# hellosunking/Microcket

Hardware: AMD Instinct MI355X
Metric: read-pairs/sec through sam2pairs+dedup (150 bp PE, hg38 names, SAM text resident in HBM) (higher is better)
Workload: dtype u8; 1 GPU; C2: 100 M 150 bp PE Micro-C read pairs, hg38, one MI355X -- 100000000 synthetic 150 bp PE read pairs per GPU, hg38 chromosome names, 1 lane(s), unc mode, sam=no, seed 20260105, one step = one pass over the whole resident data set + duplicate marking of the reported pairs on (chr1,pos1,chr2,pos2,strands) + per-chromosome-pair counts; preset=C2, pairs_per_gpu=100000001, sam_bytes_per_gpu=94584442002, block_groups=2097152, blocks=48, parallelism=shard1: independent read-group shards, no data-path collective

## Files before the change

### microcket_amd/csrc/mkt_capi.cpp

```cpp
#include "mkt_ctx.h"

extern "C" {

int mkt_abi_version(void) { return MKT_ABI_VERSION; }

const char* mkt_strerror(int code) {
    switch (code) {
    case MKT_OK: return "ok";
    case MKT_E_ARG: return "bad argument";
    case MKT_E_NO_DEVICE: return "no usable HIP device (this library has no CPU path)";
    case MKT_E_HIP: return "HIP runtime error";
    case MKT_E_NOMEM: return "out of memory";
    case MKT_E_CAPACITY: return "a QNAME group does not fit the block buffer";
    case MKT_E_KERNEL: return "kernel reported an internal error";
    case MKT_E_STATE: return "call order violated";
    case MKT_E_IO: return "temporary file error";
    default: return "unknown error";
    }
}
const char* mkt_last_error(const mkt_ctx* ctx) { return ctx ? ctx->err.c_str() : g_create_error.c_str(); }

int mkt_device_count(void) {
    int n = 0;
    if (hipGetDeviceCount(&n) != hipSuccess) return 0;
    return n;
}

static int ensure_dev(mkt_ctx* c, GrowBuf<uint8_t>& b, size_t need) { return ensure(c, b, need, need + need / 8 + 4096, true); }

static hipError_t create_device_side(mkt_ctx* c) {
    MKT_TRY(hipSetDevice(c->p.device));
    MKT_TRY(c->stream.create(hipStreamNonBlocking));
    MKT_TRY(c->d_run.alloc(1));
    MKT_TRY(hipMemsetAsync(c->d_run, 0, sizeof(DevRun), c->stream));
    MKT_TRY(c->h_res.alloc(c->res_slots));
    return hipStreamSynchronize(c->stream);
}
int mkt_create(const mkt_params* p, mkt_ctx** out) {
    if (!p || !out) return fail(nullptr, MKT_E_ARG, "null argument");
    *out = nullptr;
    if (p->mode != MKT_MODE_FLASH && p->mode != MKT_MODE_UNC) return fail(nullptr, MKT_E_ARG, "mode must be MKT_MODE_FLASH or MKT_MODE_UNC");
    if (p->ref_threads < 2) return fail(nullptr, MKT_E_ARG, "ref_threads must be >= 2 (sam2pairs.cpp:36)");
    int ndev = 0;
    if (hipGetDeviceCount(&ndev) != hipSuccess || ndev <= 0) return fail(nullptr, MKT_E_NO_DEVICE, "no HIP device: libmkt_hip has no CPU path");
    if (p->device < 0 || p->device >= ndev) return fail(nullptr, MKT_E_ARG, "device %d out of range (have %d)", p->device, ndev);
    mkt_ctx* c = new mkt_ctx();
    c->p = *p;
    c->P.mode = p->mode; c->P.ratio = p->min_mapped_ratio; c->P.min_mapq = (uint32_t)p->min_mapq; c->P.write_sam = p->write_sam ? 1 : 0;
    c->cfg = p->tiles == MKT_TILES_SMALL ? CFG_SMALL : CFG_FAST;
    c->dims = c->cfg == CFG_SMALL ? small_dims() : max_dims();
    c->dims_probed = p->tiles != MKT_TILES_AUTO || p->ordered;
    { const char* e = getenv("MKT_NO_LEAN"); c->no_lean = e && e[0] == '1'; }
    if (const char* e = getenv("MKT_FAST_ROUNDS")) {
        char* end = nullptr;
        const unsigned long v = strtoul(e, &end, 10);
        if (!strcmp(e, "all")) c->fast_rounds = 0xFFFFFFFFu;
        else if (e[0] && end && !*end && v < 0xFFFFFFFFul) c->fast_rounds = (uint32_t)v;
        else { mkt_destroy(c); return fail(nullptr, MKT_E_ARG, "MKT_FAST_ROUNDS must be a number of rounds or \"all\""); }
    }
    size_t bc = p->block_bytes ? (size_t)p->block_bytes : ((size_t)64 << 20);
    if (bc < 4096) bc = 4096;
    if (bc >= kMaxBlock) bc = kMaxBlock - 4096;
    bc = (bc + 15) & ~(size_t)15;
    c->block_cap = bc;
    c->res_slots = 1024;
    const hipError_t e = create_device_side(c);
    if (e != hipSuccess) {
        mkt_destroy(c);
        fail(nullptr, MKT_E_HIP, "mkt_create failed: %s", hipGetErrorString(e));
        return e == hipErrorOutOfMemory ? MKT_E_NOMEM : MKT_E_HIP;
    }
    *out = c;
    return MKT_OK;
}

void mkt_destroy(mkt_ctx* c) {
    if (!c) return;
    (void)hipSetDevice(c->p.device);
    if (c->worker_started) {
        { std::lock_guard<std::mutex> g(c->mu); c->stop = true; }
        c->cv.notify_all();
        c->worker.join();
    }
    (void)sync_all(c);
    delete c;
}

static int ensure_sc_list(mkt_ctx* c, size_t need);

static void set_dims_from_avg(mkt_ctx* c, double bytes_per_line) {
    c->dims_probed = true;
    c->halo_widened = 0;
    if (c->cfg == CFG_SMALL || c->p.tiles != MKT_TILES_AUTO) return;
    c->dims = lean_dims(bytes_per_line);
    if (getenv("MKT_DEBUG_SYNC")) fprintf(stderr, "tile geometry: %.1f bytes per line -> tile %u, halos %u / %u\n", bytes_per_line, c->dims.tile, c->dims.hb, c->dims.hf);
}
static bool shrink_dims(mkt_ctx* c) {
    if (c->cfg == CFG_SMALL || c->dims.tile <= 2048u) return false;
    auto f = [](uint32_t x, uint32_t lo) { uint32_t y = ((uint32_t)(x * 0.6) + 15u) & ~15u; return y < lo ? lo : y; };
    c->dims.tile = f(c->dims.tile, 2048u); c->dims.hb = f(c->dims.hb, 256u); c->dims.hf = f(c->dims.hf, 512u);
    return true;
}
static bool widen_halos(mkt_ctx* c) {
    if (c->cfg == CFG_SMALL || c->halo_widened >= 2) return false;
    const TileDims mx = max_dims();
    auto f = [](uint32_t x, uint32_t hi) { uint32_t y = ((uint32_t)(x * 1.5) + 15u) & ~15u; return y > hi ? hi : y; };
    const uint32_t hb = f(c->dims.hb, mx.hb), hf = f(c->dims.hf, mx.hf);
    const uint32_t delta = (hb - c->dims.hb) + (hf - c->dims.hf);
    if (delta == 0 || c->dims.tile < delta + 2048u) return false;
    c->dims.tile -= delta; c->dims.hb = hb; c->dims.hf = hf;
    ++c->halo_widened;
    if (getenv("MKT_DEBUG_SYNC")) fprintf(stderr, "tile geometry: halos widened -> tile %u, halos %u / %u\n", c->dims.tile, c->dims.hb, c->dims.hf);
    return true;
}
static bool adapt_geometry(mkt_ctx* c, const BlockResult& r) {
    if (c->p.tiles != MKT_TILES_AUTO || c->p.ordered) return false;
    if (r.tiles >= 1000 && (uint64_t)r.pad2 * 500 > r.tiles && widen_halos(c)) return true;
    if (r.tiles >= 8 && (uint64_t)(r.pad - r.pad2) * 8 > r.tiles) return shrink_dims(c);
    return false;
}
static double probe_device_lines(mkt_ctx* c, const uint8_t* d_text, size_t n) {
    const size_t look = n < ((size_t)1 << 20) ? n : ((size_t)1 << 20);
    if (!look) return 0;
    if (!c->h_probe && (c->d_probe.alloc(1) != hipSuccess || c->h_probe.alloc(1) != hipSuccess)) return 0;
    if (hipMemsetAsync(c->d_probe, 0, sizeof(unsigned long long), c->stream) != hipSuccess) return 0;
    if (launch_count_newlines(d_text, look, c->d_probe, c->stream) != hipSuccess) return 0;
    if (hipMemcpyAsync(c->h_probe, c->d_probe, sizeof(unsigned long long), hipMemcpyDeviceToHost, c->stream) != hipSuccess) return 0;
    if (hipStreamSynchronize(c->stream) != hipSuccess) return 0;
    return *c->h_probe ? (double)look / (double)*c->h_probe : (double)look;
}
static void smaller_geometry(mkt_ctx* c, const uint8_t* d_text, size_t n) {
    if (c->cfg != CFG_SMALL && d_text) {
        const double avg = probe_device_lines(c, d_text, n);
        const TileDims d = avg > 0 ? lean_dims(avg) : c->dims;
        if (d.tile < c->dims.tile) { c->dims = d; return; }
    }
    if (!shrink_dims(c)) { c->cfg = CFG_SMALL; c->dims = small_dims(); }
}

struct StreamOut { uint8_t* gp; size_t gp_cap; uint8_t* gs; size_t gs_cap; hipEvent_t k0, k1, done; };
static int enqueue_block(mkt_ctx* c, const uint8_t* d_text, size_t n, int cfg, const TileDims& dims, size_t slot, const StreamOut* so = nullptr) {
    if (((uintptr_t)d_text & 15u) != 0) return fail(c, MKT_E_ARG, "block text must be 16-byte aligned");
    if (n >= kMaxBlock) return fail(c, MKT_E_ARG, "block of %zu bytes: must be < 2 GiB - 64 KiB", n);
    const uint32_t ntiles = num_tiles((uint32_t)n, dims.tile);
    BlockWs ws{nullptr, ntiles};
    const size_t ws_bytes = ws.bytes();
    int rc = ensure(c, c->d_ws, ws_bytes, ws_bytes + ws_bytes / 4, true);
    if (rc) return rc;
    ws.base = c->d_ws;
    if ((ntiles + finish_chunk_tiles() - 1) / finish_chunk_tiles() > BlockWs::kScanWords) return fail(c, MKT_E_ARG, "block has too many tiles for the finish scan");
    if ((rc = ensure_dev(c, c->d_pairs, n / 3 + 65536))) return rc;
    if (c->P.write_sam && (rc = ensure_dev(c, c->d_sam, n + n / 4 + 65536))) return rc;
    if (!c->d_sc && (rc = ensure_sc_list(c, 1))) return rc;
    KArgs a;
    memset(&a, 0, sizeof a);
    a.text = d_text; a.n = (uint32_t)n; a.ntiles = ntiles; a.dims = dims; a.P = c->P;
    a.descA = ws.descA(); a.descB = ws.descB(); a.descC = ws.descC();
    a.tile_last = ws.tile_last(); a.tile_groups = ws.tile_groups(); a.defer_list = ws.defer_list();
    a.cur = ws.cur();
    a.ticket = ws.ticket(); a.defer_count = ws.defer_count(); a.fast_ticket = ws.fast_ticket();
    a.last_tile = ws.last_tile(); a.scan_ticket = ws.scan_ticket(); a.scan_desc = ws.scan_desc();
    a.res = ws.res();
    a.ordered = c->p.ordered ? 1 : 0;
    a.run = c->d_run;
    a.nregions = c->p.ordered ? 1 : kMaxRegions;
    const size_t sc_need = (size_t)a.nregions * ((n / 256 / (size_t)a.nregions) * 2 + 1024);
    if ((rc = ensure(c, c->d_sc_tmp, sc_need, sc_need, true))) return rc;
    a.pairs_rcap = (c->d_pairs.cap() / a.nregions) & ~(uint64_t)15;
    a.sam_rcap = c->P.write_sam ? ((c->d_sam.cap() / a.nregions) & ~(uint64_t)15) : 0;
    a.sc_rcap = c->d_sc_tmp.cap() / a.nregions;
    a.out.pairs = c->d_pairs; a.out.pairs_cap = c->d_pairs.cap();
    a.out.sam = c->d_sam; a.out.sam_cap = c->P.write_sam ? c->d_sam.cap() : 0;
    a.out.sc = c->d_sc_tmp; a.out.sc_cap = c->d_sc_tmp.cap();
    a.sc_list = c->d_sc; a.sc_list_cap = c->d_sc.cap();
    if (c->p.extensions & MKT_EXT_KEYS) {
        if (!c->d_chr) { HIPCHK(c, c->d_chr.alloc(1)); HIPCHK(c, hipMemsetAsync(c->d_chr, 0, sizeof(ChrTab), c->stream)); }
        const size_t per = (n / 64 / (size_t)a.nregions) * 2 + 4096, need = per * a.nregions;
        if ((rc = ensure(c, c->d_keys_raw, need, need, true))) return rc;
        const double per_byte = c->key_density > 0 ? (c->key_density * 2 < 1.0 / 64 ? c->key_density * 2 : 1.0 / 64) : 1.0 / 64;
        const size_t want = (size_t)c->acc.emitted + (size_t)((double)(c->bytes_unsynced + n) * per_byte) + 65536;
        if (!c->d_key_list.fits(want)) {
            size_t ncap = c->d_key_list.cap() ? c->d_key_list.cap() * 2 : ((size_t)1 << 22);
            while (ncap < want) ncap *= 2;
            HIPCHK(c, hipStreamSynchronize(c->stream));
            HIPCHK(c, c->d_key_list.regrow_keep(ncap, c->d_key_list.cap()));
        }
        a.keys_rcap = c->d_keys_raw.cap() / a.nregions;
        a.out.keys = c->d_keys_raw; a.out.keys_cap = c->d_keys_raw.cap(); a.out.chr = c->d_chr;
        a.out.key_lanes = (c->p.extensions & MKT_EXT_LANES) ? 1u : 0u;
        a.key_list = c->d_key_list; a.key_list_cap = c->d_key_list.cap();
    }
#if defined(MKT_STAMPS)
    if (!c->d_stamps) { HIPCHK(c, c->d_stamps.alloc(kStampWords)); HIPCHK(c, hipMemset(c->d_stamps, 0, kStampWords * sizeof(unsigned long long))); }
    a.stamps = getenv("MKT_NO_STAMPS") ? nullptr : c->d_stamps;
    { const char* e = getenv("MKT_DEBUG_STOP"); a.debug_stop = e ? atoi(e) : 0; }
#endif
    HIPCHK(c, hipMemsetAsync(c->d_ws, 0, ws_bytes, c->stream));
    hipEvent_t e0, e1;
    if (so) { e0 = so->k0; e1 = so->k1; }
    else {
        c->ev.emplace_back();
        c->ev.back().bytes = n;
        HIPCHK(c, c->ev.back().ev.create());
        e0 = c->ev.back().ev[0]; e1 = c->ev.back().ev[1];
    }
    const uint32_t max_wgs = fast_max_workgroups(cfg);
    int grid = (int)(ntiles < max_wgs ? ntiles : max_wgs);
    a.fast_dyn0 = kFastAllStatic;
    if (c->fast_rounds && ntiles > (uint32_t)grid) {
        const uint32_t rounds = ntiles / (uint32_t)grid, K = rounds > c->fast_rounds ? rounds - c->fast_rounds : 1u;
        a.fast_dyn0 = K * (uint32_t)grid;
    }
#if defined(MKT_STAMPS)
    if (a.debug_stop) a.fast_dyn0 = kFastAllStatic;
#endif
    const bool lean = !c->p.ordered && cfg != CFG_SMALL && !c->no_lean;
    HIPCHK(c, hipEventRecord(e0, c->stream));
    if (lean) {
        HIPCHK(c, launch_fast(a, cfg, grid, c->stream));
        HIPCHK(c, hipEventRecord(e1, c->stream));
        KArgs b = a;
        b.use_list = 1; b.ticket = ws.defer_ticket();
        HIPCHK(c, launch_tiles(b, cfg, ntiles < 96u ? (int)ntiles : 96, c->stream));
    } else {
        HIPCHK(c, launch_tiles(a, cfg, grid, c->stream));
        HIPCHK(c, hipEventRecord(e1, c->stream));
    }
    HIPCHK(c, launch_finish(a, c->stream));
    if (so) {
        const uint64_t prc = a.nregions > 1 ? a.pairs_rcap : 0, src_ = a.nregions > 1 ? a.sam_rcap : 0;
        HIPCHK(c, launch_gather(a.res, c->d_pairs, prc, so->gp, so->gp_cap, 0, n / 8, c->stream));
        if (c->P.write_sam) HIPCHK(c, launch_gather(a.res, c->d_sam, src_, so->gs, so->gs_cap, 1, n, c->stream));
    }
    HIPCHK(c, hipMemcpyAsync(&c->h_res[slot], a.res, sizeof(BlockResult), hipMemcpyDeviceToHost, c->stream));
    if (so) HIPCHK(c, hipEventRecord(so->done, c->stream));
    return MKT_OK;
}

static void fold_timing(mkt_ctx* c) {
    for (const mkt_ctx::Timed& t : c->ev) {
        float ms = 0;
        if (hipEventElapsedTime(&ms, t.ev[0], t.ev[1]) == hipSuccess) { c->folded_ms += ms; ++c->folded_launches; c->folded_bytes += t.bytes; }
    }
    c->ev.clear();
}

static int ensure_sc_list(mkt_ctx* c, size_t need) {
    if (c->d_sc.fits(need)) return MKT_OK;
    size_t ncap = c->d_sc.cap() ? c->d_sc.cap() : ((size_t)1 << 20);
    while (ncap < need) ncap *= 2;
    HIPCHK(c, c->d_sc.regrow_keep(ncap, c->d_sc.get() ? (size_t)c->acc.sc : 0));
    return MKT_OK;
}
static void note_sc_density(mkt_ctx* c) {
    if (c->bytes_unsynced) {
        const double d = (double)c->sc_unfolded / (double)c->bytes_unsynced;
        if (d > c->sc_density) c->sc_density = d;
        if (c->sc_density == 0) c->sc_density = 1e-12;
        const double k = (double)c->emitted_unfolded / (double)c->bytes_unsynced;
        if (k > c->key_density) c->key_density = k;
        if (c->key_density == 0) c->key_density = 1e-12;
    }
    c->sc_unfolded = 0; c->bytes_unsynced = 0; c->emitted_unfolded = 0;
}
static size_t sc_estimate(const mkt_ctx* c, size_t bytes) {
    const double per_byte = c->sc_density > 0 ? (c->sc_density * 4 > 1.0 / 65536 ? c->sc_density * 4 : 1.0 / 65536) : 1.0 / 64;
    return (size_t)((double)bytes * per_byte) + 4096;
}

static int check_result(mkt_ctx* c, const BlockResult& r) {
    if (r.err == 0) return MKT_OK;
    return fail(c, MKT_E_KERNEL, "kernel error bits 0x%x%s%s%s%s%s%s", r.err,
                (r.err & E_LINE_TABLE) ? " [line table overflow: use MKT_TILES_SMALL]" : "",
                (r.err & E_LOOKBACK) ? " [look-back timeout]" : "",
                (r.err & E_PAIRS_CAP) ? " [.pairs buffer]" : "", (r.err & E_SAM_CAP) ? " [.sam buffer]" : "",
                (r.err & E_SC_CAP) ? " [self-circle buffer]" : "", (r.err & E_FIELD_RANGE) ? " [field > 65535 bytes]" : "");
}


static int stream_start(mkt_ctx* c) {
    if (!c->s_in) HIPCHK(c, c->s_in.create(hipStreamNonBlocking));
    if (!c->s_out) HIPCHK(c, c->s_out.create(hipStreamNonBlocking));
    return MKT_OK;
}
static int stream_alloc_in(mkt_ctx* c, int i) {
    mkt_ctx::InSlot& s = c->in[i];
    if (!s.h) HIPCHK(c, s.h.alloc(c->block_cap + 64));
    return MKT_OK;
}
static int stream_alloc_dev(mkt_ctx* c, int i) {
    mkt_ctx::InSlot& s = c->in[i];
    if (!s.d) HIPCHK(c, s.d.alloc(c->block_cap + 64));
    if (!s.ev[mkt_ctx::EV_DONE]) {
        HIPCHK(c, s.ev.create(mkt_ctx::EV_H2D, hipEventDisableTiming));
        HIPCHK(c, s.ev.create(mkt_ctx::EV_K0, 0));
        HIPCHK(c, s.ev.create(mkt_ctx::EV_K1, 0));
        HIPCHK(c, s.ev.create(mkt_ctx::EV_DONE, hipEventDisableTiming));
    }
    return MKT_OK;
}
static void worker_main(mkt_ctx* c);

static int stream_launch(mkt_ctx* c, const mkt_ctx::Job& j) {
    mkt_ctx::InSlot& is = c->in[j.in_slot];
    mkt_ctx::OutSlot& os = c->outs[j.out_slot];
    int rc;
    if ((rc = ensure_dev(c, c->d_pairs, c->block_cap / 3 + 65536))) return rc;
    if (c->P.write_sam && (rc = ensure_dev(c, c->d_sam, c->block_cap + c->block_cap / 4 + 65536))) return rc;
    if ((rc = ensure_dev(c, os.d_pairs, c->d_pairs.cap()))) return rc;
    if (c->P.write_sam && (rc = ensure_dev(c, os.d_sam, c->d_sam.cap()))) return rc;
    StreamOut so;
    so.gp = os.d_pairs; so.gp_cap = os.d_pairs.cap(); so.gs = os.d_sam; so.gs_cap = os.d_sam.cap();
    so.k0 = is.ev[mkt_ctx::EV_K0]; so.k1 = is.ev[mkt_ctx::EV_K1]; so.done = is.ev[mkt_ctx::EV_DONE];
    return enqueue_block(c, is.d, j.n, j.cfg, j.dims, c->res_slots - mkt_ctx::kIn + (size_t)j.in_slot, &so);
}

static int stream_enqueue(mkt_ctx* c, std::unique_lock<std::mutex>& lk, int slot, size_t n) {
    int rc;
    if ((rc = stream_start(c))) return rc;
    const int oslot = (int)(c->seq % mkt_ctx::kOut);
    c->cv.wait(lk, [&] { return c->async_rc != MKT_OK || !c->outs[oslot].dev_busy; });
    if (c->async_rc) return c->async_rc;
    const size_t per_block = c->block_cap / 64 + 4096;
    if (!c->d_sc || (size_t)c->acc.sc + (c->jobs.size() + 1) * per_block > c->d_sc.cap()) {
        c->cv.wait(lk, [&] { return c->async_rc != MKT_OK || c->jobs.empty(); });
        if (c->async_rc) return c->async_rc;
        if ((rc = ensure_sc_list(c, 2 * (size_t)c->acc.sc + (size_t)(mkt_ctx::kOut + 1) * per_block))) return rc;
    }
    if ((rc = stream_alloc_dev(c, slot))) return rc;
    mkt_ctx::InSlot& is = c->in[slot];
    HIPCHK(c, hipMemcpyAsync(is.d, is.h, n, hipMemcpyHostToDevice, c->s_in));
    HIPCHK(c, hipEventRecord(is.ev[mkt_ctx::EV_H2D], c->s_in));
    HIPCHK(c, hipStreamWaitEvent(c->stream, is.ev[mkt_ctx::EV_H2D], 0));
    if (!c->dims_probed) {
        const size_t look = n < ((size_t)1 << 20) ? n : ((size_t)1 << 20);
        size_t lines = 0;
        for (const uint8_t* q = is.h.get(), *e = q + look; q < e && (q = (const uint8_t*)memchr(q, '\n', (size_t)(e - q))); ++q) ++lines;
        set_dims_from_avg(c, lines ? (double)look / (double)lines : (double)look);
    }
    mkt_ctx::Job j;
    j.in_slot = slot; j.out_slot = oslot; j.n = n; j.cfg = c->cfg; j.dims = c->dims; j.attempts = 0;
    c->bytes_unsynced = 0;
    for (const mkt_ctx::Job& q : c->jobs) c->bytes_unsynced += q.n;
    if ((rc = stream_launch(c, j))) return rc;
    is.busy = true; c->outs[oslot].dev_busy = true;
    c->jobs.push_back(j);
    ++c->seq;
    if (!c->worker_started) { c->worker_started = true; c->worker = std::thread(worker_main, c); }
    c->cv.notify_all();
    return MKT_OK;
}

static int rewind_run(mkt_ctx* c) {
    DevRun dr;
    dr.groups = c->acc.groups; dr.sc = c->acc.sc; dr.emitted = c->acc.emitted;
    HIPCHK(c, hipMemcpy(c->d_run, &dr, sizeof dr, hipMemcpyHostToDevice));
    return MKT_OK;
}
static int stream_replay(mkt_ctx* c, const BlockResult& r) {
    int rc;
    if ((rc = sync_all(c))) return rc;
    mkt_ctx::Job& j0 = c->jobs.front();
    if (++j0.attempts > 4) return check_result(c, r);
    bool fixed = false;
    if ((r.err & (E_LINE_TABLE | E_OVF_SLOTS)) && j0.cfg != CFG_SMALL && c->p.tiles == MKT_TILES_AUTO) {
        const int keep_cfg = c->cfg; const TileDims keep = c->dims;
        c->cfg = j0.cfg; c->dims = j0.dims;
        smaller_geometry(c, c->in[j0.in_slot].d, j0.n);
        for (mkt_ctx::Job& q : c->jobs) { q.cfg = c->cfg; q.dims = c->dims; }
        if (c->cfg == CFG_SMALL) { c->cfg = keep_cfg; c->dims = keep; }
        ++c->replays.geometry;
        fixed = true;
    } else {
        const uint32_t nr = r.nregions ? r.nregions : 1;
        if (r.err & E_PAIRS_CAP) {
            uint64_t mx = 0; for (uint32_t q = 0; q < nr; ++q) if (r.rpair[q] > mx) mx = r.rpair[q];
            if ((rc = ensure_dev(c, c->d_pairs, (size_t)(mx * nr) + mx / 4 * nr + 65536))) return rc;
            ++c->replays.pairs_cap;
            fixed = true;
        }
        if (r.err & E_SAM_CAP) {
            uint64_t mx = 0; for (uint32_t q = 0; q < nr; ++q) if (r.rsam[q] > mx) mx = r.rsam[q];
            if ((rc = ensure_dev(c, c->d_sam, (size_t)(mx * nr) + mx / 4 * nr + 65536))) return rc;
            ++c->replays.sam_cap;
            fixed = true;
        }
        if (r.err & E_SC_CAP) {
            const size_t need = (size_t)r.sc * 4 + 65536;
            HIPCHK(c, c->d_sc_tmp.regrow(need * kMaxRegions));
            if ((rc = ensure_sc_list(c, (size_t)c->acc.sc + (c->jobs.size() + 1) * need))) return rc;
            c->key_density = 0;
            ++c->replays.sc_cap;
            fixed = true;
        }
    }
    if (!fixed) return check_result(c, r);
    if ((rc = rewind_run(c))) return rc;
    c->bytes_unsynced = 0;
    for (const mkt_ctx::Job& q : c->jobs) {
        if ((rc = stream_launch(c, q))) return rc;
        c->bytes_unsynced += q.n;
        ++c->replays.jobs_rerun;
    }
    return MKT_OK;
}

static void worker_fail(mkt_ctx* c, int rc) {
    if (c->async_rc == MKT_OK) c->async_rc = rc ? rc : MKT_E_HIP;
    c->cv.notify_all();
}

static void worker_main(mkt_ctx* c) {
    (void)hipSetDevice(c->p.device);
    std::unique_lock<std::mutex> lk(c->mu);
    for (;;) {
        c->cv.wait(lk, [&] { return c->stop || (!c->jobs.empty() && c->async_rc == MKT_OK); });
        if (c->stop) return;
        const mkt_ctx::Job j = c->jobs.front();
        hipEvent_t done = c->in[j.in_slot].ev[mkt_ctx::EV_DONE];
        lk.unlock();
        hipError_t he = hipEventSynchronize(done);
        lk.lock();
        if (c->stop) return;
        if (he != hipSuccess) { fail(c, MKT_E_HIP, "hipEventSynchronize failed: %s", hipGetErrorString(he)); worker_fail(c, MKT_E_HIP); continue; }
        const BlockResult r = c->h_res[c->res_slots - mkt_ctx::kIn + (size_t)j.in_slot];
        if (r.err) {
            const int rc = stream_replay(c, r);
            if (rc) worker_fail(c, rc);
            continue;
        }
        c->acc.add_block(r); c->tiles_total += r.tiles; c->tiles_deferred += r.pad; adapt_geometry(c, r);
        ++c->blocks;
        c->sc_unfolded += r.sc; c->emitted_unfolded += r.emitted; c->bytes_unsynced = j.n;
        note_sc_density(c);
        {
            float ms = 0;
            mkt_ctx::InSlot& is = c->in[j.in_slot];
            if (hipEventElapsedTime(&ms, is.ev[mkt_ctx::EV_K0], is.ev[mkt_ctx::EV_K1]) == hipSuccess) { c->folded_ms += ms; ++c->folded_launches; c->folded_bytes += j.n; }
        }
        const size_t pb = (size_t)r.pair_bytes, sb = c->P.write_sam ? (size_t)r.sam_bytes : 0;
        mkt_ctx::OutSlot& os = c->outs[j.out_slot];
        while (os.host_busy && !c->stop) {
            if (!c->consumer_async) {
                for (mkt_ctx::Chunk& q : c->ready)
                    if (q.out_slot == j.out_slot) {
                        q.own_pairs.assign(q.pairs, q.pairs + q.pairs_len); q.own_sam.assign(q.sam, q.sam + q.sam_len);
                        q.pairs = q.own_pairs.data(); q.sam = q.own_sam.data(); q.out_slot = -1;
                    }
                if (!(c->handed_valid && c->handed.out_slot == j.out_slot)) { os.host_busy = false; break; }
            }
            c->cv.wait(lk);
        }
        if (c->stop) return;
        const size_t H = mkt_ctx::kHead;
        const size_t sam_at = ((H + pb + 4095) & ~(size_t)4095) + H, need = sam_at + sb + 64;
        bool bad = false;
        if (pb + sb) {
            const size_t want = need + need / 4;
            if (!os.h.fits(need) && os.h.regrow(want) != hipSuccess) { fail(c, MKT_E_NOMEM, "pinned staging of %zu bytes", want); worker_fail(c, MKT_E_NOMEM); bad = true; }
            if (!bad) {
                lk.unlock();
                hipError_t e1 = pb ? hipMemcpyAsync(os.h + H, os.d_pairs, pb, hipMemcpyDeviceToHost, c->s_out) : hipSuccess;
                hipError_t e2 = sb ? hipMemcpyAsync(os.h + sam_at, os.d_sam, sb, hipMemcpyDeviceToHost, c->s_out) : hipSuccess;
                hipError_t e3 = hipStreamSynchronize(c->s_out);
                lk.lock();
                if (e1 != hipSuccess || e2 != hipSuccess || e3 != hipSuccess) { fail(c, MKT_E_HIP, "output copy failed"); worker_fail(c, MKT_E_HIP); bad = true; }
            }
        }
        if (c->stop) return;
        if (bad) continue;
        mkt_ctx::Chunk ch;
        ch.out_slot = j.out_slot;
        const char* hp = (const char*)os.h.get() + H;
        const char* hs = (const char*)os.h.get() + sam_at;
        if (r.last.valid) {
            const size_t tp = r.last.pair_bytes, ts = c->P.write_sam ? r.last.sam_bytes : 0;
            const size_t bp = pb - tp, bs = sb - ts;
            ch.pairs = hp; ch.pairs_len = bp; ch.sam = hs; ch.sam_len = bs;
            if (!c->tail_pairs.empty() || !c->tail_sam.empty()) {
                if (pb + sb && c->tail_pairs.size() <= H && c->tail_sam.size() <= H) {
                    if (!c->tail_pairs.empty()) { memcpy(os.h + H - c->tail_pairs.size(), c->tail_pairs.data(), c->tail_pairs.size()); ch.pairs = hp - c->tail_pairs.size(); ch.pairs_len += c->tail_pairs.size(); }
                    if (!c->tail_sam.empty()) { memcpy(os.h + sam_at - c->tail_sam.size(), c->tail_sam.data(), c->tail_sam.size()); ch.sam = hs - c->tail_sam.size(); ch.sam_len += c->tail_sam.size(); }
                } else {
                    mkt_ctx::Chunk t;
                    t.own_pairs.swap(c->tail_pairs); t.own_sam.swap(c->tail_sam);
                    c->ready.push_back(std::move(t));
                }
            }
            if (tp) c->tail_pairs.assign(hp + bp, hp + bp + tp); else c->tail_pairs.clear();
            if (ts) c->tail_sam.assign(hs + bs, hs + bs + ts); else c->tail_sam.clear();
        } else {
            ch.pairs = hp; ch.pairs_len = pb; ch.sam = hs; ch.sam_len = sb;
        }
        if (ch.pairs_len + ch.sam_len) { os.host_busy = true; c->ready.push_back(std::move(ch)); }
        os.dev_busy = false;
        c->in[j.in_slot].busy = false;
        c->jobs.pop_front();
        c->cv.notify_all();
    }
}

static int stream_wait_idle(mkt_ctx* c, std::unique_lock<std::mutex>& lk) {
    c->cv.wait(lk, [&] { return c->async_rc != MKT_OK || c->jobs.empty(); });
    return c->async_rc;
}

static int stream_flush(mkt_ctx* c, bool everything) {
    std::unique_lock<std::mutex> lk(c->mu);
    if (c->async_rc) return c->async_rc;
    mkt_ctx::InSlot& is = c->in[c->cur];
    if (everything) {
        if (c->h_len) { int rc = stream_enqueue(c, lk, c->cur, c->h_len); if (rc) return rc; }
        c->cur = (c->cur + 1) % mkt_ctx::kIn;
        c->h_len = 0;
        return MKT_OK;
    }
    size_t end = 0;
    const size_t cut = group_aligned_prefix((const char*)is.h.get(), c->h_len, c->P.min_mapq, &end);
    if (cut == 0) {
        const size_t nl = compact_carry((char*)is.h.get(), c->h_len, c->P.min_mapq);
        if (nl + 4096 > c->h_len || nl + 4096 > c->block_cap)
            return fail(c, MKT_E_CAPACITY, "no QNAME-group boundary inside a %zu-byte block: raise block_bytes", c->block_cap);
        c->h_len = nl;
        return MKT_OK;
    }
    const int next = (c->cur + 1) % mkt_ctx::kIn;
    c->cv.wait(lk, [&] { return c->async_rc != MKT_OK || !c->in[next].busy; });
    if (c->async_rc) return c->async_rc;
    int rc = stream_alloc_in(c, next);
    if (rc) return rc;
    size_t carry = c->h_len - cut;
    memcpy(c->in[next].h, is.h + cut, carry);
    if (carry > c->block_cap / 2) carry = compact_carry((char*)c->in[next].h.get(), carry, c->P.min_mapq);
    if ((rc = stream_enqueue(c, lk, c->cur, cut))) return rc;
    c->cur = next;
    c->h_len = carry;
    return MKT_OK;
}

static int stream_check_open(mkt_ctx* c) {
    if (c->input_done || c->finished) return fail(c, MKT_E_STATE, "input after the end of input");
    { std::lock_guard<std::mutex> g(c->mu); if (c->async_rc) return c->async_rc; }
    HIPCHK(c, hipSetDevice(c->p.device));
    return stream_alloc_in(c, c->cur);
}

int mkt_submit(mkt_ctx* c, const char* bytes, size_t n, int last) {
    if (!c) return MKT_E_ARG;
    if (n && !bytes) return fail(c, MKT_E_ARG, "null bytes");
    int rc = stream_check_open(c);
    if (rc) return rc;
    size_t pos = 0;
    c->bytes_in += n;
    for (;;) {
        size_t space = c->block_cap - c->h_len;
        size_t take = n - pos < space ? n - pos : space;
        if (take) { memcpy(c->in[c->cur].h + c->h_len, bytes + pos, take); c->h_len += take; pos += take; }
        const bool all_in = pos == n;
        if (c->h_len == c->block_cap && !(all_in && last)) {
            if ((rc = stream_flush(c, false))) return rc;
            if ((rc = stream_alloc_in(c, c->cur))) return rc;
            continue;
        }
        if (all_in) break;
    }
    if (last) {
        if ((rc = stream_flush(c, true))) return rc;
        c->input_done = true;
    }
    return MKT_OK;
}

int mkt_input_window(mkt_ctx* c, char** buf, size_t* cap) {
    if (!c || !buf || !cap) return MKT_E_ARG;
    int rc = stream_check_open(c);
    if (rc) return rc;
    if (c->h_len == c->block_cap) {
        if ((rc = stream_flush(c, false))) return rc;
        if ((rc = stream_alloc_in(c, c->cur))) return rc;
    }
    *buf = (char*)c->in[c->cur].h.get() + c->h_len;
    *cap = c->block_cap - c->h_len;
    return MKT_OK;
}
int mkt_submit_window(mkt_ctx* c, size_t n, int last) {
    if (!c) return MKT_E_ARG;
    if (c->input_done || c->finished) return fail(c, MKT_E_STATE, "submit after the end of input");
    if (!c->in[c->cur].h || n > c->block_cap - c->h_len) return fail(c, MKT_E_ARG, "more bytes than the input window holds");
    HIPCHK(c, hipSetDevice(c->p.device));
    c->h_len += n;
    c->bytes_in += n;
    int rc;
    if (last) {
        if ((rc = stream_flush(c, true))) return rc;
        c->input_done = true;
    } else if (c->h_len == c->block_cap) {
        if ((rc = stream_flush(c, false))) return rc;
    }
    return MKT_OK;
}

static void release_handed(mkt_ctx* c) {
    if (c->handed_valid) {
        if (c->handed.out_slot >= 0) c->outs[c->handed.out_slot].host_busy = false;
        c->handed = mkt_ctx::Chunk();
        c->handed_valid = false;
        c->cv.notify_all();
    }
}
static void chunk_ptrs(mkt_ctx::Chunk& ch) {
    if (ch.out_slot < 0) { ch.pairs = ch.own_pairs.data(); ch.pairs_len = ch.own_pairs.size(); ch.sam = ch.own_sam.data(); ch.sam_len = ch.own_sam.size(); }
}

int mkt_drain(mkt_ctx* c, mkt_out* out) {
    if (!c || !out) return MKT_E_ARG;
    std::unique_lock<std::mutex> lk(c->mu);
    release_handed(c);
    c->drained_pairs.clear(); c->drained_sam.clear();
    while (!c->ready.empty()) {
        mkt_ctx::Chunk& ch = c->ready.front();
        chunk_ptrs(ch);
        c->drained_pairs.insert(c->drained_pairs.end(), ch.pairs, ch.pairs + ch.pairs_len);
        c->drained_sam.insert(c->drained_sam.end(), ch.sam, ch.sam + ch.sam_len);
        if (ch.out_slot >= 0) c->outs[ch.out_slot].host_busy = false;
        c->ready.pop_front();
    }
    c->cv.notify_all();
    out->pairs = c->drained_pairs.data(); out->pairs_len = c->drained_pairs.size();
    out->sam = c->drained_sam.data(); out->sam_len = c->drained_sam.size();
    return c->async_rc;
}

int mkt_drain_wait(mkt_ctx* c, mkt_out* out, int* done) {
    if (!c || !out || !done) return MKT_E_ARG;
    std::unique_lock<std::mutex> lk(c->mu);
    release_handed(c);
    memset(out, 0, sizeof *out);
    *done = 0;
    c->consumer_async = true;
    c->cv.wait(lk, [&] { return c->async_rc != MKT_OK || !c->ready.empty() || c->finished; });
    if (!c->ready.empty()) {
        c->handed = std::move(c->ready.front());
        c->ready.pop_front();
        c->handed_valid = true;
        chunk_ptrs(c->handed);
        out->pairs = c->handed.pairs; out->pairs_len = c->handed.pairs_len; out->sam = c->handed.sam; out->sam_len = c->handed.sam_len;
        return MKT_OK;
    }
    *done = 1;
    return c->async_rc;
}

int mkt_submit_device(mkt_ctx* c, const void* d_text, size_t n) {
    if (!c) return MKT_E_ARG;
    if (c->finished) return fail(c, MKT_E_STATE, "submit after finish");
    if (!d_text && n) return fail(c, MKT_E_ARG, "null device pointer");
    HIPCHK(c, hipSetDevice(c->p.device));
    const bool probe = c->probing && c->res_used >= 1;
    if (probe || c->res_used == c->res_slots - mkt_ctx::kIn || (size_t)c->acc.sc + sc_estimate(c, c->bytes_unsynced + n) > c->d_sc.cap()) {
        if (getenv("MKT_DEBUG_SYNC")) fprintf(stderr, "submit_device: sync before block (slots %zu/%zu, unsynced %.1f GB, density %.3g /B, list %llu of %zu)\n",
                                              c->res_used, c->res_slots, (double)c->bytes_unsynced / 1e9, c->sc_density, (unsigned long long)c->acc.sc, c->d_sc.cap());
        int rc = mkt_sync(c);
        if (rc) return rc;
        if ((rc = ensure_sc_list(c, 2 * (size_t)c->acc.sc + sc_estimate(c, n)))) return rc;
    }
    if (!c->dims_probed) {
        const double avg = probe_device_lines(c, (const uint8_t*)d_text, n);
        if (avg <= 0 && n) return fail(c, MKT_E_HIP, "line-length probe failed: %s", hipGetErrorString(hipGetLastError()));
        set_dims_from_avg(c, avg);
    }
    c->bytes_unsynced += n;
    const int cfg_used = c->cfg;
    const TileDims dims_used = c->dims;
    int rc = enqueue_block(c, (const uint8_t*)d_text, n, cfg_used, dims_used, c->res_used);
    if (rc) return rc;
    if (c->res_text.size() < c->res_slots) { c->res_text.resize(c->res_slots); c->res_n.resize(c->res_slots); }
    c->res_text[c->res_used] = (const uint8_t*)d_text; c->res_n[c->res_used] = n;
    ++c->res_used;
    c->last_n = n; c->last_dims = dims_used; c->last_text = (const uint8_t*)d_text;
    c->bytes_in += n;
    return MKT_OK;
}

int mkt_sync(mkt_ctx* c) {
    if (!c) return MKT_E_ARG;
    HIPCHK(c, hipSetDevice(c->p.device));
    { std::unique_lock<std::mutex> lk(c->mu); const int arc = stream_wait_idle(c, lk); if (arc) return arc; }
    const bool dbg = getenv("MKT_DEBUG_SYNC") != nullptr;
    auto now = [] { return std::chrono::duration<double, std::milli>(std::chrono::steady_clock::now().time_since_epoch()).count(); };
    const double t0 = dbg ? now() : 0;
    HIPCHK(c, hipStreamSynchronize(c->stream));
    const double t1 = dbg ? now() : 0;
    fold_timing(c);
    const double t2 = dbg ? now() : 0;
    int rc = MKT_OK;
    bool changed = false;
    int replays = 0;
    for (size_t k = c->res_folded; k < c->res_used; ++k) {
        const BlockResult& r = c->h_res[k];
        if (r.err) {
            if ((r.err & (E_LINE_TABLE | E_OVF_SLOTS)) && c->p.tiles == MKT_TILES_AUTO && c->cfg != CFG_SMALL && replays < 4 && c->res_text.size() > k) {
                ++replays;
                ++c->replays.geometry; c->replays.jobs_rerun += c->res_used - k;
                smaller_geometry(c, c->res_text[k], c->res_n[k]);
                c->last_dims = c->dims;
                changed = true;
                if ((rc = rewind_run(c))) return rc;
                for (size_t j = k; j < c->res_used; ++j) if ((rc = enqueue_block(c, c->res_text[j], c->res_n[j], c->cfg, c->dims, j))) return rc;
                HIPCHK(c, hipStreamSynchronize(c->stream));
                fold_timing(c);
                --k;
                continue;
            }
            rc = check_result(c, r);
            break;
        }
        c->acc.add_block(r); c->tiles_total += r.tiles; c->tiles_deferred += r.pad;
        changed = adapt_geometry(c, r) || changed;
        c->sc_unfolded += r.sc; c->emitted_unfolded += r.emitted;
        ++c->blocks;
    }
    if (c->res_used > c->res_folded) c->probing = changed;
    const size_t nres = c->res_used;
    c->res_used = 0; c->res_folded = 0;
    if (rc == MKT_OK) note_sc_density(c);
    if (dbg) fprintf(stderr, "mkt_sync: %zu blocks, wait %.2f ms, timing fold %.2f ms, results %.2f ms\n", nres, t1 - t0, t2 - t1, now() - t2);
    return rc;
}

int mkt_fetch_last_block(mkt_ctx* c, char* pairs, size_t pairs_cap, size_t* pairs_len, char* sam, size_t sam_cap, size_t* sam_len) {
    if (!c) return MKT_E_ARG;
    HIPCHK(c, hipSetDevice(c->p.device));
    HIPCHK(c, hipStreamSynchronize(c->stream));
    BlockResult r;
    const uint32_t ntiles = num_tiles((uint32_t)c->last_n, c->last_dims.tile ? c->last_dims.tile : c->dims.tile);
    HIPCHK(c, hipMemcpy(&r, BlockWs{c->d_ws, ntiles}.res(), sizeof r, hipMemcpyDeviceToHost));
    if (pairs_len) *pairs_len = (size_t)r.pair_bytes;
    if (sam_len) *sam_len = c->P.write_sam ? (size_t)r.sam_bytes : 0;
    const uint32_t nreg = r.nregions ? r.nregions : 1;
    const size_t prc = (c->d_pairs.cap() / nreg) & ~(size_t)15, src_ = c->P.write_sam ? ((c->d_sam.cap() / nreg) & ~(size_t)15) : 0;
    if (pairs && r.pair_bytes) {
        if (pairs_cap < r.pair_bytes) return fail(c, MKT_E_ARG, "pairs buffer too small (%llu needed)", (unsigned long long)r.pair_bytes);
        size_t acc = 0;
        for (uint32_t q = 0; q < nreg; ++q) { if (r.rpair[q]) HIPCHK(c, hipMemcpy(pairs + acc, c->d_pairs + (size_t)q * prc, (size_t)r.rpair[q], hipMemcpyDeviceToHost)); acc += (size_t)r.rpair[q]; }
    }
    if (sam && c->P.write_sam && r.sam_bytes) {
        if (sam_cap < r.sam_bytes) return fail(c, MKT_E_ARG, "sam buffer too small (%llu needed)", (unsigned long long)r.sam_bytes);
        size_t acc = 0;
        for (uint32_t q = 0; q < nreg; ++q) { if (r.rsam[q]) HIPCHK(c, hipMemcpy(sam + acc, c->d_sam + (size_t)q * src_, (size_t)r.rsam[q], hipMemcpyDeviceToHost)); acc += (size_t)r.rsam[q]; }
    }
    return MKT_OK;
}

int mkt_finish(mkt_ctx* c, int drop_last, uint64_t group_offset, uint64_t total_groups, mkt_stats* st) {
    if (!c || !st) return MKT_E_ARG;
    int rc = mkt_sync(c);
    if (rc) return rc;
    const uint64_t K = total_groups ? total_groups : c->acc.groups;
    unsigned long long logged = 0;
    if (c->acc.sc) {
        if (!c->d_sc_logged) HIPCHK(c, c->d_sc_logged.alloc(1));
        HIPCHK(c, hipMemsetAsync(c->d_sc_logged, 0, sizeof(unsigned long long), c->stream));
        const uint64_t drop_group = c->acc.drops(drop_last != 0) ? c->acc.groups - 1 : ~0ull;
        HIPCHK(c, launch_sc_logged(c->d_sc, c->acc.sc, drop_group, group_offset, K, (uint32_t)c->p.ref_threads, c->d_sc_logged, c->stream));
        HIPCHK(c, hipMemcpyAsync(&logged, c->d_sc_logged, sizeof logged, hipMemcpyDeviceToHost, c->stream));
        HIPCHK(c, hipStreamSynchronize(c->stream));
    }
    RunStats s = c->acc.finish_logged(drop_last != 0, logged);
    memset(st, 0, sizeof *st);
    st->lowMap = s.counters[C_LOWMAP]; st->manyHits = s.counters[C_MANYHITS]; st->unpaired = s.counters[C_UNPAIRED];
    st->selfCircle = s.counters[C_SELFCIRCLE]; st->trans = s.counters[C_TRANS];
    st->cis10K = s.counters[C_CIS10K]; st->cis1K = s.counters[C_CIS1K]; st->cis0 = s.counters[C_CIS0];
    st->selfCircle_all = s.selfcircle_all;
    st->groups = s.groups; st->pairs = s.pairs; st->pair_bytes = s.pair_bytes; st->sam_bytes = s.sam_bytes;
    st->bytes_in = c->bytes_in; st->blocks = c->blocks;
    {
        std::lock_guard<std::mutex> g(c->mu);
        if (!c->finished) {
            if (!drop_last && (!c->tail_pairs.empty() || !c->tail_sam.empty())) {
                mkt_ctx::Chunk t;
                t.own_pairs.swap(c->tail_pairs); t.own_sam.swap(c->tail_sam);
                c->ready.push_back(std::move(t));
            }
            c->tail_pairs.clear(); c->tail_sam.clear();
            c->finished = true;
        }
    }
    c->cv.notify_all();
    return MKT_OK;
}

int mkt_reset(mkt_ctx* c) {
    if (!c) return MKT_E_ARG;
    HIPCHK(c, hipSetDevice(c->p.device));
    {
        std::unique_lock<std::mutex> lk(c->mu);
        c->cv.wait(lk, [&] { return c->async_rc != MKT_OK || c->jobs.empty(); });
        (void)sync_all(c);
        c->jobs.clear(); c->ready.clear(); c->handed = mkt_ctx::Chunk(); c->handed_valid = false;
        for (int i = 0; i < mkt_ctx::kIn; ++i) c->in[i].busy = false;
        for (int i = 0; i < mkt_ctx::kOut; ++i) { c->outs[i].dev_busy = false; c->outs[i].host_busy = false; }
        c->async_rc = MKT_OK; c->cur = 0; c->seq = 0; c->consumer_async = false;
    }
    HIPCHK(c, hipStreamSynchronize(c->stream));
    fold_timing(c);
    HIPCHK(c, hipMemsetAsync(c->d_run, 0, sizeof(DevRun), c->stream));
    HIPCHK(c, hipStreamSynchronize(c->stream));
    c->acc = RunAccum();
    c->sc_unfolded = 0; c->bytes_unsynced = 0; c->emitted_unfolded = 0;
    c->sc_density = 0; c->key_density = 0; c->probing = true;
    c->dims_probed = c->p.tiles != MKT_TILES_AUTO || c->p.ordered || c->cfg == CFG_SMALL;
    if (c->d_chr) HIPCHK(c, hipMemsetAsync(c->d_chr, 0, sizeof(ChrTab), c->stream));
    c->res_used = c->res_folded = 0;
    c->h_len = 0;
    c->tail_pairs.clear(); c->tail_sam.clear(); c->drained_pairs.clear(); c->drained_sam.clear();
    c->input_done = c->finished = false;
    c->bytes_in = 0; c->blocks = 0;
    return MKT_OK;
}

int mkt_format_log(const mkt_stats* st, char* out, size_t cap) {
    if (!st || !out) return MKT_E_ARG;
    return snprintf(out, cap, "lowMap\t%u\nmanyHits\t%u\nunpaired\t%u\nselfCircle\t%u\ntrans\t%u\ncis10K\t%u\ncis1K\t%u\ncis0\t%u\n",
                    st->lowMap, st->manyHits, st->unpaired, st->selfCircle, st->trans, st->cis10K, st->cis1K, st->cis0);
}

int mkt_get_timing(const mkt_ctx* c, mkt_timing* t) {
    if (!c || !t) return MKT_E_ARG;
    t->tile_kernel_ms = c->folded_ms; t->tile_launches = c->folded_launches; t->tile_bytes = c->folded_bytes; t->other_ms = 0;
    t->tiles = c->tiles_total; t->deferred_tiles = c->tiles_deferred;
    return MKT_OK;
}
int mkt_reset_timing(mkt_ctx* c) {
    if (!c) return MKT_E_ARG;
    c->folded_ms = 0; c->folded_launches = 0; c->folded_bytes = 0; c->tiles_total = 0; c->tiles_deferred = 0;
    std::lock_guard<std::mutex> g(c->mu);
    c->replays = mkt_replays{0, 0, 0, 0, 0};
    return MKT_OK;
}
int mkt_get_replays(const mkt_ctx* c, mkt_replays* r) {
    if (!c || !r) return MKT_E_ARG;
    std::lock_guard<std::mutex> g(const_cast<mkt_ctx*>(c)->mu);
    *r = c->replays;
    return MKT_OK;
}

}
```

### microcket_amd/csrc/mkt_capi_util.cpp

```cpp
#include "mkt_ctx.h"
#include <memory>

extern "C" {

int mkt_synth_device(mkt_ctx* c, uint64_t seed, int profile, int genome, int read_len, int lanes, uint64_t first_group,
                     uint64_t n_groups, int tail_group, const void** d_text, size_t* n_bytes) {
    if (!c || !d_text || !n_bytes) return MKT_E_ARG;
    HIPCHK(c, hipSetDevice(c->p.device));
    SynParams sp;
    sp.seed = seed; sp.profile = profile; sp.genome = genome; sp.read_len = read_len; sp.lanes = lanes;
    int rc = ensure(c, c->d_syn_sizes, n_groups + 2, n_groups + 2, false);
    if (rc) return rc;
    uint64_t* d_total = c->d_syn_sizes + n_groups;
    HIPCHK(c, launch_synth_sizes(sp, first_group, n_groups, c->d_syn_sizes, c->stream));
    HIPCHK(c, launch_exscan(c->d_syn_sizes, n_groups, d_total, c->stream));
    uint64_t total = 0;
    HIPCHK(c, hipMemcpyAsync(&total, d_total, sizeof total, hipMemcpyDeviceToHost, c->stream));
    HIPCHK(c, hipStreamSynchronize(c->stream));
    size_t tail = tail_group ? synth_tail_bytes(sp) : 0;
    size_t need = (size_t)total + tail + 64;
    if ((rc = ensure(c, c->d_syn, need, need, false))) return rc;
    HIPCHK(c, launch_synth_write(sp, first_group, n_groups, c->d_syn_sizes, c->d_syn, c->stream));
    if (tail) HIPCHK(c, launch_synth_tail(sp, c->d_syn + total, c->stream));
    HIPCHK(c, hipStreamSynchronize(c->stream));
    *d_text = c->d_syn;
    *n_bytes = (size_t)total + tail;
    return MKT_OK;
}

struct mkt_dataset {
    mkt_ctx* ctx;
    DevBuf<char> arena;
    std::vector<uint64_t> off, len, groups;
    uint64_t total_bytes = 0, total_groups = 0;
};

int mkt_dataset_create(mkt_ctx* c, uint64_t seed, int profile, int genome, int read_len, int lanes, uint64_t first_group,
                       uint64_t n_groups, uint64_t gpb, int tail_group, mkt_dataset** out) {
    if (!c || !out || gpb == 0) return MKT_E_ARG;
    *out = nullptr;
    HIPCHK(c, hipSetDevice(c->p.device));
    SynParams sp;
    sp.seed = seed; sp.profile = profile; sp.genome = genome; sp.read_len = read_len; sp.lanes = lanes;
    const int rc = ensure(c, c->d_syn_sizes, gpb + 2, gpb + 2, false);
    if (rc) return rc;
    std::unique_ptr<mkt_dataset> ds(new mkt_dataset());
    ds->ctx = c;
    const uint64_t nb = (n_groups + gpb - 1) / gpb;
    const size_t tail = tail_group ? synth_tail_bytes(sp) : 0;
    uint64_t* d_total = c->d_syn_sizes + gpb;
    uint64_t cursor = 0;
    for (uint64_t b = 0; b < nb; ++b) {
        const uint64_t g0 = b * gpb, g = (g0 + gpb <= n_groups) ? gpb : n_groups - g0;
        HIPCHK(c, launch_synth_sizes(sp, first_group + g0, g, c->d_syn_sizes, c->stream));
        HIPCHK(c, launch_exscan(c->d_syn_sizes, g, d_total, c->stream));
        uint64_t total = 0;
        HIPCHK(c, hipMemcpyAsync(&total, d_total, sizeof total, hipMemcpyDeviceToHost, c->stream));
        HIPCHK(c, hipStreamSynchronize(c->stream));
        if (b + 1 == nb) total += tail;
        if (total >= kMaxBlock) return fail(c, MKT_E_ARG, "block %llu would hold %llu bytes (>= 2 GiB - 64 KiB): lower groups_per_block", (unsigned long long)b, (unsigned long long)total);
        ds->off.push_back(cursor); ds->len.push_back(total); ds->groups.push_back(g + ((b + 1 == nb && tail_group) ? 1 : 0));
        cursor += (total + 15) & ~(uint64_t)15;
    }
    ds->total_bytes = 0;
    for (uint64_t l : ds->len) ds->total_bytes += l;
    ds->total_groups = n_groups + (tail_group ? 1 : 0);
    const hipError_t e = ds->arena.alloc(cursor + 64);
    if (e != hipSuccess) return fail(c, MKT_E_NOMEM, "hipMalloc of %llu bytes for the data set failed: %s", (unsigned long long)cursor, hipGetErrorString(e));
    for (uint64_t b = 0; b < nb; ++b) {
        const uint64_t g0 = b * gpb, g = (g0 + gpb <= n_groups) ? gpb : n_groups - g0;
        HIPCHK(c, launch_synth_sizes(sp, first_group + g0, g, c->d_syn_sizes, c->stream));
        HIPCHK(c, launch_exscan(c->d_syn_sizes, g, d_total, c->stream));
        HIPCHK(c, launch_synth_write(sp, first_group + g0, g, c->d_syn_sizes, ds->arena + ds->off[b], c->stream));
        if (b + 1 == nb && tail) HIPCHK(c, launch_synth_tail(sp, ds->arena + ds->off[b] + ds->len[b] - tail, c->stream));
        HIPCHK(c, hipStreamSynchronize(c->stream));
    }
    *out = ds.release();
    return MKT_OK;
}
int mkt_dataset_info(const mkt_dataset* ds, uint64_t* n_blocks, uint64_t* total_bytes, uint64_t* total_groups) {
    if (!ds) return MKT_E_ARG;
    if (n_blocks) *n_blocks = ds->off.size();
    if (total_bytes) *total_bytes = ds->total_bytes;
    if (total_groups) *total_groups = ds->total_groups;
    return MKT_OK;
}
int mkt_dataset_block(const mkt_dataset* ds, uint64_t i, const void** d_text, size_t* n_bytes, uint64_t* n_groups) {
    if (!ds || i >= ds->off.size()) return MKT_E_ARG;
    if (d_text) *d_text = ds->arena + ds->off[i];
    if (n_bytes) *n_bytes = (size_t)ds->len[i];
    if (n_groups) *n_groups = ds->groups[i];
    return MKT_OK;
}
void mkt_dataset_destroy(mkt_dataset* ds) {
    if (!ds) return;
    (void)hipSetDevice(ds->ctx->p.device);
    delete ds;
}

int mkt_group_count(mkt_ctx* c, uint64_t* groups) {
    if (!c || !groups) return MKT_E_ARG;
    int rc = mkt_sync(c);
    if (rc) return rc;
    *groups = c->acc.groups;
    return MKT_OK;
}

#if defined(MKT_STAMPS)
int mkt_debug_stamps(mkt_ctx* c, unsigned long long* out16) {
    if (!c || !out16) return MKT_E_ARG;
    memset(out16, 0, 16 * sizeof(unsigned long long));
    if (!c->d_stamps) return MKT_OK;
    HIPCHK(c, hipStreamSynchronize(c->stream));
    HIPCHK(c, hipMemcpy(out16, c->d_stamps, 16 * sizeof(unsigned long long), hipMemcpyDeviceToHost));
    HIPCHK(c, hipMemset(c->d_stamps, 0, 16 * sizeof(unsigned long long)));
    return MKT_OK;
}
int mkt_debug_spans(mkt_ctx* c, unsigned long long* out4) {
    if (!c || !out4) return MKT_E_ARG;
    memset(out4, 0, 4 * sizeof(unsigned long long));
    if (!c->d_stamps) return MKT_OK;
    HIPCHK(c, hipStreamSynchronize(c->stream));
    HIPCHK(c, hipMemcpy(out4, c->d_stamps + 16, 4 * sizeof(unsigned long long), hipMemcpyDeviceToHost));
    HIPCHK(c, hipMemset(c->d_stamps + 16, 0, 4 * sizeof(unsigned long long)));
    return MKT_OK;
}
#endif

int mkt_device_text(mkt_ctx* c, const char* bytes, size_t n, const void** d_text) {
    if (!c || !d_text || (n && !bytes)) return MKT_E_ARG;
    HIPCHK(c, hipSetDevice(c->p.device));
    c->uploads.emplace_back();
    HIPCHK(c, c->uploads.back().alloc(n + 64));
    uint8_t* d = c->uploads.back();
    if (n) HIPCHK(c, hipMemcpy(d, bytes, n, hipMemcpyHostToDevice));
    *d_text = d;
    return MKT_OK;
}

int mkt_copy_to_host(mkt_ctx* c, const void* d_src, void* dst, size_t n) {
    if (!c || !d_src || !dst) return MKT_E_ARG;
    HIPCHK(c, hipSetDevice(c->p.device));
    HIPCHK(c, hipMemcpy(dst, d_src, n, hipMemcpyDeviceToHost));
    return MKT_OK;
}

}
```

### microcket_amd/csrc/mkt_ctx.h

```cpp
#pragma once
#include <hip/hip_runtime.h>
#include <stdarg.h>
#include <stdio.h>
#include <stdlib.h>
#include <string.h>
#include <algorithm>
#include <string>
#include <utility>
#include <chrono>
#include <condition_variable>
#include <deque>
#include <mutex>
#include <thread>
#include <vector>

#include "../../include/mkt.h"
#include "mkt_launch.h"
#include "mkt_devbuf.h"

using namespace mkt;

static const size_t kMaxBlock = ((size_t)1 << 31) - 65536;
static const uint32_t kFastRoundsDefault = 8;
static const size_t kStampWords = 20;

inline thread_local std::string g_create_error;

struct mkt_ctx {
    mkt_params p;
    Params P;
    DevStream stream, s_in, s_out;
    int cfg = CFG_FAST;
    TileDims dims = {0, 0, 0};
    bool dims_probed = false;
    DevBuf<unsigned long long> d_probe; PinBuf<unsigned long long> h_probe;
    TileDims last_dims = {0, 0, 0};
    const uint8_t* last_text = nullptr;
    bool probing = true;
    size_t block_cap = 0;
    GrowBuf<uint8_t> d_pairs, d_sam;
    GrowBuf<uint64_t> d_sc;
    DevBuf<unsigned long long> d_sc_logged;
    PinBuf<uint8_t> h_chr_stage; DevBuf<uint16_t> d_dense;
    GrowBuf<uint8_t> d_dd_flags, d_dd_work;
    DevBuf<DedupResult> d_dd_res; PinBuf<DedupResult> h_dd_res;
    GrowBuf<uint32_t> d_perm; DevBuf<uint32_t> d_part_hist; DevBuf<uint16_t> d_lut; uint64_t part_n = 0;
    GrowBuf<unsigned long long> d_chr_counts; PinGrowBuf<unsigned long long> h_chr_counts;
    double sc_density = 0;
    GrowBuf<uint64_t> d_sc_tmp;
    GrowBuf<KeyRec> d_keys_raw;
    GrowBuf<KeyRec> d_key_list;
    DevBuf<ChrTab> d_chr;
    GrowBuf<uint8_t> d_ws;
    DevBuf<DevRun> d_run;
    size_t h_len = 0;
    PinBuf<BlockResult> h_res; size_t res_slots = 0, res_used = 0, res_folded = 0;
    std::vector<DevBuf<uint8_t>> uploads;
    std::vector<const uint8_t*> res_text; std::vector<size_t> res_n;
    static constexpr int kIn = 3, kOut = 2;
    static constexpr size_t kHead = 65536;
    enum { EV_H2D, EV_K0, EV_K1, EV_DONE };
    struct InSlot { PinBuf<uint8_t> h; DevBuf<uint8_t> d; bool busy = false; DevEvents<4> ev; };
    struct OutSlot { GrowBuf<uint8_t> d_pairs, d_sam; PinGrowBuf<uint8_t> h; bool dev_busy = false, host_busy = false; };
    struct Job { int in_slot, out_slot; size_t n; int cfg; TileDims dims; int attempts; };
    struct Chunk { const char* pairs = nullptr; size_t pairs_len = 0; const char* sam = nullptr; size_t sam_len = 0; int out_slot = -1;
                   std::vector<char> own_pairs, own_sam; };
    InSlot in[kIn];
    OutSlot outs[kOut];
    std::deque<Job> jobs;
    std::deque<Chunk> ready;
    Chunk handed; bool handed_valid = false;
    std::mutex mu;
    std::condition_variable cv;
    std::thread worker;
    bool worker_started = false, stop = false;
    int async_rc = MKT_OK;
    bool consumer_async = false;
    int cur = 0;
    uint64_t seq = 0;
    std::vector<char> tail_pairs, tail_sam, drained_pairs, drained_sam;
    RunAccum acc;
    bool input_done = false, finished = false;
    uint64_t bytes_in = 0, blocks = 0;
    size_t last_n = 0;
    double key_density = 0;
    uint64_t emitted_unfolded = 0;
    uint64_t sc_unfolded = 0;
    uint64_t bytes_unsynced = 0;
    struct Timed { DevEvents<2> ev; uint64_t bytes = 0; };
    std::deque<Timed> ev;
    double folded_ms = 0; uint64_t folded_launches = 0, folded_bytes = 0;
    uint64_t tiles_total = 0, tiles_deferred = 0;
    mkt_replays replays = {0, 0, 0, 0, 0};
    GrowBuf<char> d_syn;
    GrowBuf<uint64_t> d_syn_sizes;
    DevBuf<unsigned long long> d_stamps;
    uint32_t fast_rounds = kFastRoundsDefault;
    bool no_lean = false;
    int halo_widened = 0;
    std::string err;
};

inline int fail(mkt_ctx* c, int code, const char* fmt, ...) {
    char buf[512];
    va_list ap;
    va_start(ap, fmt);
    vsnprintf(buf, sizeof buf, fmt, ap);
    va_end(ap);
    if (c) c->err = buf; else g_create_error = buf;
    return code;
}
#define HIPCHK(c, call)                                                                            \
    do {                                                                                           \
        hipError_t e_ = (call);                                                                    \
        if (e_ != hipSuccess) return fail((c), MKT_E_HIP, "%s failed: %s", #call, hipGetErrorString(e_)); \
    } while (0)

inline int sync_all(mkt_ctx* c) {
    if (c->s_in) HIPCHK(c, hipStreamSynchronize(c->s_in));
    if (c->stream) HIPCHK(c, hipStreamSynchronize(c->stream));
    if (c->s_out) HIPCHK(c, hipStreamSynchronize(c->s_out));
    return MKT_OK;
}
template <typename B>
inline int ensure(mkt_ctx* c, B& buf, size_t need, size_t new_cap, bool sync) {
    if (buf.fits(need)) return MKT_OK;
    if (sync && buf.get()) { const int rc = sync_all(c); if (rc) return rc; }
    HIPCHK(c, buf.regrow(new_cap));
    return MKT_OK;
}
inline uint64_t ext_key_count(mkt_ctx* c, int drop_last) {
    uint64_t n = c->acc.emitted;
    if (drop_last && c->acc.pending.valid && c->acc.pending.pair_bytes && n) --n;
    return n;
}
```

### microcket_amd/csrc/mkt_kernels.hip

```cpp
#include <hip/hip_runtime.h>
#include <type_traits>
#include "mkt_launch.h"

namespace mkt {

constexpr int NT = 256;
constexpr uint64_t FLAG_AGG = 1ull << 62, FLAG_PREFIX = 2ull << 62, PAYLOAD = (1ull << 62) - 1;
constexpr uint32_t LOOKBACK_SPIN_LIMIT = 1u << 22;

struct ScanScratch { uint64_t a[NT / 64], b[NT / 64]; };

#if defined(MKT_STAMPS)
#define STAMP_DECL() unsigned long long stamp_prev_ = 0, stamp_first_ = 0, stamp_acc_[16] = {0, 0, 0, 0, 0, 0, 0, 0, 0, 0, 0, 0, 0, 0, 0, 0}
#define STAMP(k)                                                                        \
    do {                                                                                \
        if (tid == 0 && a.stamps) {                                                     \
            const unsigned long long now_ = __builtin_amdgcn_s_memtime();               \
            if ((k) > 0) stamp_acc_[(k)] += now_ - stamp_prev_;                         \
            else if (!stamp_first_) stamp_first_ = __builtin_amdgcn_s_memrealtime();   \
            stamp_prev_ = now_;                                                         \
        }                                                                               \
    } while (0)
#define STAMP_SPAN(t0_)                                                                 \
    do {                                                                                \
        if ((t0_) == 0 && a.stamps && stamp_first_) {                                   \
            const unsigned long long end_ = __builtin_amdgcn_s_memrealtime();           \
            atomicAdd(&a.stamps[16], end_ - stamp_first_); atomicMax(&a.stamps[17], end_ - stamp_first_); \
            atomicMax(&a.stamps[18], end_); atomicMax(&a.stamps[19], (1ull << 62) - stamp_first_); \
        }                                                                               \
    } while (0)
#define STAMP_FLUSH(t0_)                                                                \
    do {                                                                                \
        if ((t0_) == 0 && a.stamps) for (int k_ = 1; k_ < 16; ++k_) if (stamp_acc_[k_]) atomicAdd(&a.stamps[k_], stamp_acc_[k_]); \
    } while (0)
#define STOP_AFTER(k) if (a.debug_stop == (k)) { __syncthreads(); continue; }
#else
#define STAMP_DECL() do { } while (0)
#define STAMP(k) do { } while (0)
#define STAMP_FLUSH(t0_) do { } while (0)
#define STAMP_SPAN(t0_) do { } while (0)
#define STOP_AFTER(k)
#endif

__device__ inline uint64_t shfl_up64(uint64_t v, int d) { return (uint64_t)__shfl_up((long long)v, d, 64); }
__device__ inline uint64_t shfl_xor64(uint64_t v, int d) { return (uint64_t)__shfl_xor((long long)v, d, 64); }

__device__ inline void block_exscan1(uint32_t& a, uint32_t& total, ScanScratch& sc) {
    const int lane = threadIdx.x & 63, wv = threadIdx.x >> 6;
    uint32_t ia = a;
#pragma unroll
    for (int d = 1; d < 64; d <<= 1) {
        const uint32_t x = (uint32_t)__shfl_up((int)ia, d, 64);
        if (lane >= d) ia += x;
    }
    if (lane == 63) sc.a[wv] = ia;
    __syncthreads();
    uint32_t pre = 0;
    total = 0;
#pragma unroll
    for (int w = 0; w < NT / 64; ++w) {
        const uint32_t x = (uint32_t)sc.a[w];
        if (w < wv) pre += x;
        total += x;
    }
    a = pre + ia - a;
    __syncthreads();
}

__device__ inline uint32_t wave_iscan32(uint32_t v) {
    v += (uint32_t)__builtin_amdgcn_update_dpp(0, (int)v, 0x111, 0xF, 0xF, false);
    v += (uint32_t)__builtin_amdgcn_update_dpp(0, (int)v, 0x112, 0xF, 0xF, false);
    v += (uint32_t)__builtin_amdgcn_update_dpp(0, (int)v, 0x114, 0xF, 0xF, false);
    v += (uint32_t)__builtin_amdgcn_update_dpp(0, (int)v, 0x118, 0xF, 0xF, false);
    v += (uint32_t)__builtin_amdgcn_update_dpp(0, (int)v, 0x142, 0xA, 0xF, false);
    v += (uint32_t)__builtin_amdgcn_update_dpp(0, (int)v, 0x143, 0xC, 0xF, false);
    return v;
}
template <int NW>
__device__ inline void block_exscan3(uint32_t& a, uint32_t& b, uint32_t& c, uint32_t& ta, uint32_t& tb, uint32_t& tc, ScanScratch& sc) {
    const int lane = threadIdx.x & 63, wv = threadIdx.x >> 6;
    const uint32_t ia = wave_iscan32(a), ib = wave_iscan32(b), ic = wave_iscan32(c);
    if (lane == 63) { sc.a[wv] = (uint64_t)ia | ((uint64_t)ib << 32); sc.b[wv] = ic; }
    __syncthreads();
    uint32_t pa = 0, pb = 0, pc = 0;
    ta = 0; tb = 0; tc = 0;
#pragma unroll
    for (int w = 0; w < NW; ++w) {
        const uint64_t x = sc.a[w];
        const uint32_t xa = (uint32_t)x, xb = (uint32_t)(x >> 32), xc = (uint32_t)sc.b[w];
        if (w < wv) { pa += xa; pb += xb; pc += xc; }
        ta += xa; tb += xb; tc += xc;
    }
    a = pa + ia - a; b = pb + ib - b; c = pc + ic - c;
}

__device__ inline void block_exscan2(uint64_t& a, uint64_t& b, uint64_t& ta, uint64_t& tb, ScanScratch& sc) {
    const int lane = threadIdx.x & 63, wv = threadIdx.x >> 6;
    uint64_t ia = a, ib = b;
#pragma unroll
    for (int d = 1; d < 64; d <<= 1) {
        uint64_t xa = shfl_up64(ia, d), xb = shfl_up64(ib, d);
        if (lane >= d) { ia += xa; ib += xb; }
    }
    if (lane == 63) { sc.a[wv] = ia; sc.b[wv] = ib; }
    __syncthreads();
    uint64_t pa = 0, pb = 0;
    ta = 0; tb = 0;
#pragma unroll
    for (int w = 0; w < NT / 64; ++w) {
        if (w < wv) { pa += sc.a[w]; pb += sc.b[w]; }
        ta += sc.a[w]; tb += sc.b[w];
    }
    a = pa + ia - a;
    b = pb + ib - b;
    __syncthreads();
}

__device__ inline uint32_t zero_bytes(uint32_t x) { return ~(((x & 0x7F7F7F7Fu) + 0x7F7F7F7Fu) | x | 0x7F7F7F7Fu); }
__device__ inline uint32_t ge_bytes(uint32_t x, uint32_t n) { return (((x & 0x7F7F7F7Fu) + (0x80u - n) * 0x01010101u) | x) & 0x80808080u; }
__device__ inline uint32_t pack_msb(uint32_t z) { return (((z >> 7) * 0x00204081u) >> 21) & 0xFu; }
__device__ inline uint32_t nl_bits(uint32_t x) { return pack_msb(zero_bytes(x ^ 0x0A0A0A0Au)); }
__device__ inline uint32_t ws_bits(uint32_t x) {
    const uint32_t ctl = ge_bytes(x, 9u) & ~ge_bytes(x, 14u);
    return pack_msb(ctl | zero_bytes(x ^ 0x20202020u));
}

__device__ inline uint32_t nl_flags(uint32_t x) {
    const uint32_t y = x & 0x7F7F7F7Fu;
    return ~((y ^ 0x0A0A0A0Au) + 0x7F7F7F7Fu) & ~x & 0x80808080u;
}
__device__ inline uint32_t has_nl(uint32_t x) {
    const uint32_t t = x ^ 0x0A0A0A0Au;
    return (t - 0x01010101u) & ~t & 0x80808080u;
}
__device__ inline uint32_t sep_flags(uint32_t x) {
    const uint32_t y = x & 0x7F7F7F7Fu;
    return ~((y + 0x5F5F5F5Fu) | x) & 0x80808080u;
}
__device__ inline uint32_t pack16(uint32_t f0, uint32_t f1, uint32_t f2, uint32_t f3) {
    const uint32_t lo = __builtin_amdgcn_udot4(f1, 0x80402010u, __builtin_amdgcn_udot4(f0, 0x08040201u, 0u, false), false);
    const uint32_t hi = __builtin_amdgcn_udot4(f3, 0x80402010u, __builtin_amdgcn_udot4(f2, 0x08040201u, 0u, false), false);
    return (lo >> 7) | ((hi >> 7) << 8);
}

__device__ inline uint64_t lookback(uint64_t* desc, uint32_t t, uint64_t agg, uint32_t* err_word) {
    const int lane = threadIdx.x & 63;
    if (t == 0) {
        if (lane == 0) __hip_atomic_store(&desc[0], FLAG_PREFIX | agg, __ATOMIC_RELAXED, __HIP_MEMORY_SCOPE_AGENT);
        return 0;
    }
    if (lane == 0) __hip_atomic_store(&desc[t], FLAG_AGG | agg, __ATOMIC_RELAXED, __HIP_MEMORY_SCOPE_AGENT);
    uint64_t excl = 0;
    int64_t j = (int64_t)t - 1;
    uint32_t spins = 0;
    for (;;) {
        const int64_t idx = j - lane;
        uint64_t w = FLAG_PREFIX;
        if (idx >= 0) w = __hip_atomic_load(&desc[idx], __ATOMIC_RELAXED, __HIP_MEMORY_SCOPE_AGENT);
        const uint32_t flag = (uint32_t)(w >> 62);
        const uint64_t m_prefix = __ballot(flag == 2);
        const uint64_t m_invalid = __ballot(flag == 0);
        const int first = m_prefix ? __builtin_ctzll(m_prefix) : 64;
        const uint64_t needed = first >= 63 ? ~0ull : ((1ull << (first + 1)) - 1);
        if (m_invalid & needed) {
            if (++spins > LOOKBACK_SPIN_LIMIT) { if (lane == 0) atomicOr(err_word, (uint32_t)E_LOOKBACK); break; }
            __builtin_amdgcn_s_sleep(4);
            continue;
        }
        uint64_t c = lane <= first ? (w & PAYLOAD) : 0;
#pragma unroll
        for (int d = 32; d >= 1; d >>= 1) c += shfl_xor64(c, d);
        excl += c;
        if (first < 64) break;
        j -= 64;
    }
    if (lane == 0) __hip_atomic_store(&desc[t], FLAG_PREFIX | ((excl + agg) & PAYLOAD), __ATOMIC_RELAXED, __HIP_MEMORY_SCOPE_AGENT);
    return excl;
}

__device__ inline uint32_t claim_ranges(const KArgs& a, uint32_t region, const TileSums& sums, TileSums& base,
                                        uint32_t& region_pair0, uint32_t& region_sam0, OutPtrs& lim) {
    RegionCur* cur = a.cur + region;
    uint32_t err = 0;
    const uint64_t p0 = (uint64_t)region * a.pairs_rcap, s0 = (uint64_t)region * a.sam_rcap, c0 = (uint64_t)region * a.sc_rcap;
    unsigned long long oa = 0, ob = 0;
    if (sums.pair_bytes | sums.emitted) oa = atomicAdd(&cur->a, (unsigned long long)sums.pair_bytes | ((unsigned long long)sums.emitted << kCurShift));
    if (sums.sam_bytes | sums.sc) ob = atomicAdd(&cur->b, (unsigned long long)sums.sam_bytes | ((unsigned long long)sums.sc << kCurShift));
    const uint64_t op = oa & kCurLow, os = ob & kCurLow, oc = ob >> kCurShift;
    if (op + sums.pair_bytes > a.pairs_rcap) err |= E_PAIRS_CAP;
    if (os + sums.sam_bytes > a.sam_rcap) err |= E_SAM_CAP;
    if (oc + sums.sc > a.sc_rcap) err |= E_SC_CAP;
    base.pair_bytes = (uint32_t)(p0 + op); base.sam_bytes = s0 + os; base.sc = (uint32_t)(c0 + oc);
    base.emitted = (uint32_t)((uint64_t)region * a.keys_rcap + (oa >> kCurShift));
    lim.keys_cap = a.keys_rcap ? ((uint64_t)region * a.keys_rcap + ((oa >> kCurShift) + sums.emitted <= a.keys_rcap ? a.keys_rcap : 0)) : 0;
    region_pair0 = (uint32_t)p0; region_sam0 = (uint32_t)s0;
    lim.pairs_cap = err & E_PAIRS_CAP ? 0 : p0 + a.pairs_rcap;
    lim.sam_cap = err & E_SAM_CAP ? 0 : s0 + a.sam_rcap;
    lim.sc_cap = err & E_SC_CAP ? 0 : c0 + a.sc_rcap;
    return err;
}

template <class Cfg>
__global__ __launch_bounds__(NT) void k_tiles(KArgs a) {
    __shared__ TileState<Cfg> st;
    __shared__ ScanScratch scan;
    __shared__ uint32_t s_tile;
    constexpr int NVEC = (Cfg::W + 15) / 16;
    constexpr int NM16 = Cfg::MW * 4;
    constexpr int VPT = (NVEC + NT - 1) / NT;
    constexpr int IPT = (Cfg::LCAP + NT - 1) / NT;
    const int tid = threadIdx.x;
    const Params P = a.P;
    const uint32_t n = a.n;
    __shared__ OutPtrs s_out;
    const uint32_t region = a.nregions > 1 ? (blockIdx.x & (uint32_t)(a.nregions - 1)) : 0u;
    uint16_t* nlmask = reinterpret_cast<uint16_t*>(st.u.m.nlm);
    uint16_t* wsmask = reinterpret_cast<uint16_t*>(st.u.m.wsm);
    STAMP_DECL();

    for (;;) {
        if (tid == 0) {
            s_out = a.out;
            uint32_t k = atomicAdd(a.ticket, 1u);
            if (a.use_list) k = k < *a.defer_count ? a.defer_list[k] : 0xFFFFFFFFu;
            s_tile = k;
            tile_reset(st);
        }
        __syncthreads();
        const uint32_t t = s_tile;
        if (t >= a.ntiles) break;
        STAMP(0);
        const TileGeom G = tile_geom(t, n, a.dims);
        const uint32_t wlen = G.w1 - G.w0;
        const uint32_t nvec = (wlen + 15u) >> 4;
        const TextView tv = tile_view(st, a.text, n, G);

        constexpr int SPT = (NM16 + NT - 1) / NT;
        uint4 xs[SPT];
#pragma unroll
        for (int q = 0; q < SPT; ++q) {
            const uint32_t v = (uint32_t)tid + (uint32_t)q * NT;
            const uint32_t go = G.w0 + (v << 4);
            xs[q] = *reinterpret_cast<const uint4*>(a.text + ((v < nvec && go + 16u <= n) ? go : 0u));
        }
#pragma unroll
        for (int q = 0; q < SPT; ++q) {
            const uint32_t v = (uint32_t)tid + (uint32_t)q * NT;
            if (v >= (uint32_t)NM16) continue;
            uint32_t mnl = 0, mws = 0;
            if (v < nvec) {
                const uint32_t go = G.w0 + (v << 4);
                uint4 x;
                if (go + 16u <= n) {
                    x = xs[q];
                } else {
                    uint32_t w[4] = {0, 0, 0, 0};
                    for (uint32_t b = 0; go + b < n; ++b) w[b >> 2] |= (uint32_t)a.text[go + b] << ((b & 3u) * 8u);
                    x = make_uint4(w[0], w[1], w[2], w[3]);
                }
                *reinterpret_cast<uint4*>(&st.win[v << 4]) = x;
                mnl = nl_bits(x.x) | (nl_bits(x.y) << 4) | (nl_bits(x.z) << 8) | (nl_bits(x.w) << 12);
                mws = ws_bits(x.x) | (ws_bits(x.y) << 4) | (ws_bits(x.z) << 8) | (ws_bits(x.w) << 12);
                const uint32_t r0 = v << 4;
                if (r0 + 16u > wlen) {
                    const uint32_t keep = wlen - r0;
                    mnl &= (1u << keep) - 1u; mws &= (1u << keep) - 1u;
                }
            } else if (v == nvec && (v << 4) < (uint32_t)(Cfg::W + 16)) {
                *reinterpret_cast<uint4*>(&st.win[v << 4]) = make_uint4(0, 0, 0, 0);
            }
            nlmask[v] = (uint16_t)mnl;
            wsmask[v] = (uint16_t)mws;
        }
        __syncthreads();
        STAMP(1);

        {
            uint64_t cnt = 0, dummy = 0, total, td;
            const uint32_t v0 = tid * VPT;
            auto line_bits = [&](uint32_t v) -> uint32_t {
                uint32_t m = nlmask[v];
                const uint32_t r0 = v << 4;
                if (r0 + 16u > wlen - 1u) { const uint32_t keep = wlen - 1u > r0 ? wlen - 1u - r0 : 0u; m &= keep >= 16u ? 0xFFFFu : ((1u << keep) - 1u); }
                return m;
            };
            for (uint32_t k = 0; k < (uint32_t)VPT; ++k) if (v0 + k < nvec) cnt += __popc(line_bits(v0 + k));
            uint64_t ex = cnt;
            block_exscan2(ex, dummy, total, td, scan);
            const uint32_t lead = G.w0 == 0 ? 1u : 0u;
            const uint32_t NL = (uint32_t)total + lead;
            if (NL > (uint32_t)Cfg::LCAP) {
                if (tid == 0) { lds_or(&st.err, E_LINE_TABLE); st.NL = 0; st.first_idx = 0; st.end_idx = 0; }
            } else {
                uint32_t idx = (uint32_t)ex + lead;
                for (uint32_t k = 0; k < (uint32_t)VPT; ++k) {
                    if (v0 + k >= nvec) break;
                    uint32_t m = line_bits(v0 + k);
                    while (m) {
                        const uint32_t b = __builtin_ctz(m);
                        st.off[idx++] = G.w0 + ((v0 + k) << 4) + b + 1u;
                        m &= m - 1u;
                    }
                }
                if (tid == 0) { if (lead) st.off[0] = 0; st.NL = NL; st.first_idx = NL; st.end_idx = NL; }
            }
        }
        __syncthreads();
        const uint32_t NL = st.NL;

        STAMP(2);
        for (uint32_t i = tid; i < NL; i += NT) ph_parse(st, tv, P, G, i);
        __syncthreads();
        if (tid == 0) tile_trim(st);
        __syncthreads();
        STAMP(3);
        const uint32_t first_idx = st.first_idx, end_idx = st.end_idx;
        for (uint32_t i = first_idx + tid; i < end_idx; i += NT) ph_group(st, tv, P, G, i);
        __syncthreads();
        STAMP(4);
        STAMP(5);

        {
            auto& g = st.u.g;
            uint64_t ca = 0, cb = 0;
            const uint32_t i0 = first_idx + tid * IPT;
            for (uint32_t k = 0; k < (uint32_t)IPT; ++k) {
                const uint32_t i = i0 + k;
                if (i >= end_idx) break;
                const uint32_t info = g.g_info[i];
                if (info & GI_START) ca += 1ull;
                if (info & GI_EMIT) ca += 1ull << 16;
                if ((info & GI_START) && (info & GI_COUNTER) == C_SELFCIRCLE) ca += 1ull << 32;
                cb += (uint64_t)g.g_plen[i] | ((uint64_t)g.g_slen[i] << 32);
            }
            uint64_t ea = ca, eb = cb, ta, tb;
            block_exscan2(ea, eb, ta, tb, scan);
            for (uint32_t k = 0; k < (uint32_t)IPT; ++k) {
                const uint32_t i = i0 + k;
                if (i >= end_idx) break;
                g.x_grp[i] = (uint16_t)(ea & 0xFFFFu); g.x_sc[i] = (uint16_t)((ea >> 32) & 0xFFFFu); g.x_emit[i] = (uint16_t)((ea >> 16) & 0xFFFFu);
                g.x_pair[i] = (uint32_t)eb; g.x_sam[i] = (uint32_t)(eb >> 32);
                const uint32_t info = g.g_info[i];
                if (info & GI_EMIT) g.em_idx[(ea >> 16) & 0xFFFFu] = (uint16_t)i;
                if (info & GI_START) ea += 1ull;
                if (info & GI_EMIT) ea += 1ull << 16;
                if ((info & GI_START) && (info & GI_COUNTER) == C_SELFCIRCLE) ea += 1ull << 32;
                eb += (uint64_t)g.g_plen[i] | ((uint64_t)g.g_slen[i] << 32);
            }
            if (tid == 0) {
                st.sums.groups = (uint32_t)(ta & 0xFFFFu); st.sums.emitted = (uint32_t)((ta >> 16) & 0xFFFFu); st.sums.sc = (uint32_t)((ta >> 32) & 0xFFFFu);
                st.sums.pair_bytes = (uint32_t)tb; st.sums.sam_bytes = tb >> 32;
            }
        }
        __syncthreads();
        STAMP(6);
        if (a.ordered) {
            const int wv = tid >> 6;
            if (wv == 0) {
                uint64_t ex = lookback(a.descA, t, ((uint64_t)st.sums.groups << 31) | st.sums.emitted, &a.res->err);
                if ((tid & 63) == 0) { st.base.groups = (uint32_t)(ex >> 31); st.base.emitted = (uint32_t)(ex & 0x7FFFFFFFu); }
            } else if (wv == 1) {
                uint64_t ex = lookback(a.descB, t, ((uint64_t)st.sums.pair_bytes << 31) | st.sums.sc, &a.res->err);
                if ((tid & 63) == 0) { st.base.pair_bytes = (uint32_t)(ex >> 31); st.base.sc = (uint32_t)(ex & 0x7FFFFFFFu); }
            } else if (wv == 2) {
                uint64_t ex = lookback(a.descC, t, st.sums.sam_bytes, &a.res->err);
                if ((tid & 63) == 0) st.base.sam_bytes = ex;
            } else if (tid == 192) {
                if (st.sums.pair_bytes | st.sums.emitted) atomicAdd(&a.cur[0].a, (unsigned long long)st.sums.pair_bytes | ((unsigned long long)st.sums.emitted << kCurShift));
                if (st.sums.sam_bytes | st.sums.sc) atomicAdd(&a.cur[0].b, (unsigned long long)st.sums.sam_bytes | ((unsigned long long)st.sums.sc << kCurShift));
            }
        } else if (tid == 0) {
            const uint32_t e = claim_ranges(a, region, st.sums, st.base, st.region_pair0, st.region_sam0, s_out);
            st.region_id = region;
            if (e) lds_or(&st.err, e);
        }
        if (tid == 5) a.tile_groups[t] = (uint64_t)st.sums.groups | ((uint64_t)st.sums.emitted << 32);
        __syncthreads();
        STAMP(7);

        for (uint32_t i = first_idx + tid; i < end_idx; i += NT) {
            ph_account(st, tv, P, s_out, t, i);
            ph_last(st, &a.tile_last[t], i);
        }
        {
            const uint32_t total = st.sums.pair_bytes;
            const uint64_t go = st.base.pair_bytes;
            if (go + total <= s_out.pairs_cap) { for (uint32_t e = tid; e < st.sums.emitted; e += NT) tile_emit_line(st, tv, e, s_out.pairs + go); }
            else if (tid == 0 && total) lds_or(&st.err, E_PAIRS_CAP);
        }
        if (P.write_sam) {
            for (uint32_t i = first_idx; i < end_idx; ++i) {
                const uint32_t info = st.u.g.g_info[i];
                if ((info & (GI_EMIT | GI_CONTIG)) != (GI_EMIT | GI_CONTIG)) continue;
                const uint32_t len = st.u.g.g_slen[i], src = st.off[i];
                const uint64_t go = st.base.sam_bytes + st.u.g.x_sam[i];
                if (go + len <= s_out.sam_cap) { for (uint32_t k = tid; k < len; k += NT) s_out.sam[go + k] = tv.at(src + k); }
                else if (tid == 0) lds_or(&st.err, E_SAM_CAP);
            }
        }
        __syncthreads();
        STAMP(8);
        if (tid < (int)C_COUNT && st.cnt[tid]) atomicAdd(&a.res->counters[tid], st.cnt[tid]);
        if (tid == 0 && st.err) atomicOr(&a.res->err, st.err);
        __syncthreads();
    }
    STAMP_FLUSH(tid);
}

constexpr int kLoadBatch = 14;
__device__ inline uint32_t nl_xad(uint32_t y, uint32_t nl, uint32_t m1) {
    uint32_t r;
    asm("v_xad_u32 %0, %1, %2, %3" : "=v"(r) : "v"(y), "s"(nl), "v"(m1));
    return r;
}
struct NlConst { uint32_t nl, m1; };
__device__ inline NlConst nl_const() {
    NlConst c;
    c.nl = 0x0A0A0A0Au; c.m1 = 0xFEFEFEFFu;
    asm volatile("" : "+s"(c.nl));
    asm volatile("" : "+v"(c.m1));
    return c;
}
__device__ inline uint64_t has_newline_ballot(const uint4& y, bool valid, const NlConst& c) {
    const uint32_t nl = c.nl, m1 = c.m1;
    const uint32_t r0 = __builtin_amdgcn_bitop3_b32(nl_xad(y.x, nl, m1), y.x, nl, 0x90), r1 = __builtin_amdgcn_bitop3_b32(nl_xad(y.y, nl, m1), y.y, nl, 0x90);
    const uint32_t r2 = __builtin_amdgcn_bitop3_b32(nl_xad(y.z, nl, m1), y.z, nl, 0x90), r3 = __builtin_amdgcn_bitop3_b32(nl_xad(y.w, nl, m1), y.w, nl, 0x90);
    const uint32_t z = __builtin_amdgcn_bitop3_b32(__builtin_amdgcn_bitop3_b32(r0, r1, r2, 0xFE), r3, 0x80808080u, 0xA8);
    return __ballot(z != 0u && valid);
}
template <class Cfg, uint32_t nws>
__device__ inline void fast_scan(const KArgs& a, uint32_t tt, uint64_t* hit, uint32_t ws_, uint32_t kb, uint32_t ke, int lane) {
    const uint32_t ws = (uint32_t)__builtin_amdgcn_readfirstlane((int)ws_);
    const NlConst nlc = nl_const();
    const uint32_t n = a.n;
    const TileGeom G = tile_geom(tt, n, a.dims);
    const uint32_t wlen = G.w1 - G.w0, nvec = (wlen + 15u) >> 4;
    const uint8_t* wbase = a.text + G.w0;
    const uint32_t loff = (uint32_t)lane << 4;
    const uint32_t ngr = nvec >> 6;
    if (!(wlen & 1023u) && kb < ke && (ke - 1u) * nws + ws < ngr && ke - kb <= (uint32_t)kLoadBatch) {
        const uint32_t cnt = ke - kb, stride = nws << 10;
        const uint8_t* p0 = wbase + ((size_t)(kb * nws + ws) << 10);
        uint4 x[kLoadBatch];
#pragma unroll
        for (int k = 0; k < kLoadBatch; ++k) {
            const uint32_t kk = (uint32_t)k < cnt ? (uint32_t)k : cnt - 1u;
            x[k] = *reinterpret_cast<const uint4*>(p0 + (size_t)kk * stride + loff);
        }
#pragma unroll
        for (int k = 0; k < kLoadBatch; ++k) {
            if ((uint32_t)k < cnt) {
                const uint64_t bm = has_newline_ballot(x[k], true, nlc);
                const uint32_t g = (kb + (uint32_t)k) * nws + ws;
                if (lane == 0 && g < (uint32_t)Cfg::HMW) hit[g] = bm;
            }
        }
        return;
    }
    const uint32_t tail = (G.w1 >= n) ? (wlen & 15u) : 0u;
    for (uint32_t k0 = kb; k0 < ke; k0 += kLoadBatch) {
        uint4 x[kLoadBatch];
#pragma unroll
        for (int k = 0; k < kLoadBatch; ++k) {
            const uint32_t g0 = (k0 + k) * nws + ws, glast = (nvec - 1u) >> 6, g = g0 < glast ? g0 : glast;
            const uint32_t lim = nvec - (g << 6), l = (uint32_t)lane < lim ? (uint32_t)lane : lim - 1u;
            x[k] = *reinterpret_cast<const uint4*>(wbase + ((size_t)g << 10) + (l << 4));
        }
#pragma unroll
        for (int k = 0; k < kLoadBatch; ++k) {
            const uint32_t g = (k0 + k) * nws + ws;
            if (k0 + k >= ke || (g << 6) >= nvec) continue;
            uint4 y = x[k];
            if (tail && (g << 6) + 64u >= nvec && (g << 6) + (uint32_t)lane == nvec - 1u) {
                uint32_t* w = reinterpret_cast<uint32_t*>(&y);
#pragma unroll
                for (int d = 0; d < 4; ++d) {
                    const uint32_t lo = (uint32_t)d * 4u;
                    w[d] = tail >= lo + 4u ? w[d] : (tail > lo ? (w[d] & ((1u << ((tail - lo) * 8u)) - 1u)) : 0u);
                }
            }
            const uint64_t bm = has_newline_ballot(y, (uint32_t)lane < nvec - (g << 6), nlc);
            if (lane == 0 && g < (uint32_t)Cfg::HMW) hit[g] = bm;
        }
    }
}

template <class Cfg, int NTW, int RR, int WPS>
__global__ __launch_bounds__(NTW, WPS) void k_fast(KArgs a) {
    __shared__ FastState<Cfg> st;
    __shared__ ScanScratch scan;
    static_assert(Cfg::LCAP <= NTW, "one line per thread in the sums");
    static_assert(NTW % 64 == 0 && NTW <= NT && RR * 64 <= NTW, "whole waves");
    const int tid0 = threadIdx.x;
    const Params P = a.P;
    const uint32_t n = a.n;
    __shared__ OutPtrs s_out;
    const uint32_t region = blockIdx.x & (uint32_t)(a.nregions - 1);
    STAMP_DECL();

    __shared__ uint32_t wg_cnt[C_COUNT];
    __shared__ uint64_t s_hit[2][Cfg::HMW + 1];
    constexpr int NWV = NTW / 64;
    constexpr int NSW = NWV >= 4 ? 2 : 0;
    const uint32_t ngrp = (a.dims.hb + a.dims.tile + a.dims.hf + 1023u) >> 10;
    const uint32_t lpt_all = (ngrp + NWV - 1) / NWV, lpt_sw = NSW ? (ngrp + NSW - 1) / NSW : 0u, lpt_a = (lpt_sw + 1u) >> 1;
    auto own = [&](uint32_t ws, uint32_t nws, uint32_t ke) { const uint32_t c = ws < ngrp ? (ngrp - ws + nws - 1u) / nws : 0u; return ke < c ? ke : c; };
    if (tid0 < (int)C_COUNT) wg_cnt[tid0] = 0;
    fast_init(st, (uint32_t)tid0);
    if (tid0 == 0) s_out = a.out;
    uint32_t gdim = gridDim.x;
    asm volatile("" : "+s"(gdim));
    __shared__ uint32_t s_next[2];
    const bool ticket_lane = tid0 == NTW - 64;
    if (blockIdx.x + gdim >= a.fast_dyn0) {
        if (ticket_lane) s_next[0] = a.fast_dyn0 + atomicAdd(a.fast_ticket, 1u);
        __syncthreads();
    }
    auto next_of = [&](uint32_t x, uint32_t c) { return x + gdim < a.fast_dyn0 ? x + gdim : (uint32_t)__builtin_amdgcn_readfirstlane((int)s_next[c]); };
    uint32_t cur = 0;
    bool scanned = false;
    for (uint32_t t = blockIdx.x; t < a.ntiles; t = next_of(t, cur ^ 1u)) {
        int tid = tid0;
        asm volatile("" : "+v"(tid));
        if (tid == 0) fast_reset(st);
        STAMP(0);
        const TileGeom G = tile_geom(t, n, a.dims);
        const TextView tv = fast_view(st, a.text, n, G);

        const uint32_t wave = (uint32_t)__builtin_amdgcn_readfirstlane(tid >> 6);
        if (!scanned) fast_scan<Cfg, NWV>(a, t, s_hit[cur], wave, 0u, own(wave, NWV, lpt_all), tid & 63);
        scanned = false;
        __syncthreads();
        STAMP(1);
        STOP_AFTER(1)

        if (tid < 64) {
            static_assert(Cfg::HMW <= 64, "one bitmap word per lane of one wave");
            uint64_t m = (uint32_t)tid < ((G.w1 - G.w0 + 1023u) >> 10) ? s_hit[cur][tid] : 0ull;
            const uint32_t cnt = (uint32_t)__popcll(m);
            const uint32_t inc = wave_iscan32(cnt);
            const uint32_t total = (uint32_t)__builtin_amdgcn_readlane((int)inc, 63);
            const uint32_t lead = G.w0 == 0 ? 1u : 0u;
            const uint32_t NLt = total + lead;
            if (NLt > (uint32_t)Cfg::LCAP) {
                if (tid == 0) { st.abn = AB_LCAP; st.NL = 0; }
            } else {
                uint32_t idx = inc - cnt + lead;
                while (m) {
                    st.hv16[idx++] = (uint16_t)(((uint32_t)tid << 6) + (uint32_t)__builtin_ctzll(m));
                    m &= m - 1ull;
                }
                if (tid == 0) {
                    if (lead) st.hv16[0] = 0;
                    st.NL = NLt; st.first_idx = NLt; st.end_idx = NLt;
                    st.last_line_end = G.w1 >= n ? n : kUnknown;
                }
            }
        }
        __syncthreads();
        const uint32_t NL = st.NL;
        STAMP(2);
        STOP_AFTER(2)
        {
            constexpr int HPT = (Cfg::LCAP * Cfg::HCH + NTW - 1) / NTW;
            auto heads = [&](auto edge_c) {
                constexpr bool EDGE = decltype(edge_c)::value;
                uint4 q[HPT];
#pragma unroll
                for (int k = 0; k < HPT; ++k) {
                    const uint32_t it = (uint32_t)tid + (uint32_t)k * NTW;
                    q[k] = make_uint4(0, 0, 0, 0);
                    if (it < NL * (uint32_t)Cfg::HCH) {
                        const uint32_t i = it / (uint32_t)Cfg::HCH, c = it % (uint32_t)Cfg::HCH;
                        const uint32_t g0 = G.w0 + (((uint32_t)st.hv16[i] + c) << 4);
                        if (!EDGE || g0 < n) q[k] = *reinterpret_cast<const uint4*>(a.text + g0);
                    }
                }
#pragma unroll
                for (int k = 0; k < HPT; ++k) {
                    const uint32_t it = (uint32_t)tid + (uint32_t)k * NTW;
                    if (it >= NL * (uint32_t)Cfg::HCH) continue;
                    const uint32_t i = it / (uint32_t)Cfg::HCH, c = it % (uint32_t)Cfg::HCH;
                    uint4 x = q[k];
                    uint32_t keep = 16u;
                    if (EDGE) {
                        const uint32_t g0 = G.w0 + (((uint32_t)st.hv16[i] + c) << 4);
                        keep = g0 >= n ? 0u : (n - g0 < 16u ? n - g0 : 16u);
                        if (keep != 0u && keep < 16u) {
                            uint32_t* w = reinterpret_cast<uint32_t*>(&x);
#pragma unroll
                            for (int d = 0; d < 4; ++d) {
                                const uint32_t lo = (uint32_t)d * 4u;
                                w[d] = keep >= lo + 4u ? w[d] : (keep > lo ? (w[d] & ((1u << ((keep - lo) * 8u)) - 1u)) : 0u);
                            }
                        }
                    }
                    {
                        uint32_t* row = reinterpret_cast<uint32_t*>(&st.win[mul24(i, (uint32_t)Cfg::HSTRIDE) + (c << 4)]);
                        row[0] = x.x; row[1] = x.y; row[2] = x.z; row[3] = x.w;
                    }
                    uint32_t m = pack16(sep_flags(x.x), sep_flags(x.y), sep_flags(x.z), sep_flags(x.w));
                    if (EDGE && keep < 16u) m &= (1u << keep) - 1u;
                    st.u.m.hmask[i][c] = (uint16_t)m;
                }
            };
            if ((uint64_t)G.w1 + 16u * ((uint32_t)Cfg::HCH + 2u) > (uint64_t)n) heads(std::true_type{});
            else heads(std::false_type{});
        }
        __syncthreads();
        STAMP(9);
        STOP_AFTER(9)

        const uint32_t ltid = (uint32_t)tid;
        const uint32_t rr_id = ((uint32_t)tid >> 6) < (uint32_t)RR ? ((uint32_t)tid & 63u) * RR + ((uint32_t)tid >> 6) : 0xFFFFFFu;
        {
            const uint32_t i = ltid;
            uint32_t lb = 0, fl = 0;
            if (i < NL) { fast_parse(st, tv, P, G, i); lb = st.bits[i]; fl = st.flag[i]; }
            const bool sv = (lb & LB_SURVIVE) != 0;
            const uint64_t b_s = __ballot(sv), b_e = __ballot((lb & LB_EQPREV) != 0);
            const uint64_t b_1 = __ballot(sv && (fl & 64u)), b_2 = __ballot(sv && !(fl & 64u) && (fl & 128u));
            const uint32_t gs = i < NL ? (uint32_t)st.goff[i] : 0u;
            const uint64_t b_t0 = __ballot(i < NL && G.w0 + gs >= G.t0), b_t1 = __ballot(i < NL && G.w0 + gs >= G.t1);
            if ((tid & 63) == 0) {
                const uint32_t w = ltid >> 6; st.m_surv[w] = b_s; st.m_eqp[w] = b_e; st.m_r1[w] = b_1; st.m_r2[w] = b_2;
                if (b_t0) atomicAdd(&st.c_t0, (uint32_t)__popcll(b_t0));
                if (b_t1) atomicAdd(&st.c_t1, (uint32_t)__popcll(b_t1));
            }
            if (NTW < 256 && tid < 4 && tid >= NTW / 64) { st.m_surv[tid] = 0; st.m_eqp[tid] = 0; st.m_r1[tid] = 0; st.m_r2[tid] = 0; st.m_start[tid] = 0; }
        }
        if (NSW && wave >= (uint32_t)(NWV - NSW)) {
            const uint32_t nxt = next_of(t, cur);
            if (nxt < a.ntiles)
                fast_scan<Cfg, (NSW ? NSW : 1)>(a, nxt, s_hit[cur ^ 1u], wave - (uint32_t)(NWV - NSW), 0u, own(wave - (uint32_t)(NWV - NSW), NSW, lpt_a), tid & 63);
        }
        __syncthreads();
        STAMP(3);
        STOP_AFTER(3)
        const uint32_t NLe = fast_nle(st);
        const uint32_t first_idx = NL - st.c_t0 < NLe ? NL - st.c_t0 : NLe;
        const uint32_t end_idx = NL - st.c_t1 < NLe ? NL - st.c_t1 : NLe;
        {
            const uint32_t i = ltid;
            bool s0 = false;
            if (!st.abn && i >= first_idx && i < NLe && mask_bit(st.m_surv, i)) s0 = fast_is_start(st, tv, G, i);
            const uint64_t b = __ballot(s0);
            if ((tid & 63) == 0) st.m_start[ltid >> 6] = b;
        }
        __syncthreads();
        STAMP(10);
#if defined(MKT_STAMPS)
        if (a.debug_stop == 10) {
            if (a.out.sam && !st.abn) for (uint32_t i = first_idx + (uint32_t)tid; i < end_idx; i += NTW) {
                const uint4 r0 = make_uint4(st.rc.f.pos[i], st.rc.f.lclip[i] | (st.rc.f.rclip[i] << 16), st.rc.f.mappable[i] | ((uint32_t)st.flag[i] << 16), st.rc.f.right0[i]);
                const uint4 r1 = make_uint4(st.rc.f.left1[i], st.rc.f.right1[i], G.w0 + st.goff[i], st.qn_len[i] | ((uint32_t)st.rn_off[i] << 8) | ((uint32_t)st.rn_len[i] << 16) | ((uint32_t)st.bits[i] << 24));
                uint4* d = reinterpret_cast<uint4*>(a.out.sam + ((size_t)t * Cfg::LCAP + i) * 32u);
                if (((size_t)t * Cfg::LCAP + i) * 32u + 32u <= a.out.sam_cap) { d[0] = r0; d[1] = r1; }
            }
            const uint32_t nxt = next_of(t, cur);
            if (NSW && wave >= (uint32_t)(NWV - NSW) && nxt < a.ntiles)
                fast_scan<Cfg, (NSW ? NSW : 1)>(a, nxt, s_hit[cur ^ 1u], wave - (uint32_t)(NWV - NSW), lpt_a, own(wave - (uint32_t)(NWV - NSW), NSW, lpt_sw), tid & 63);
            scanned = NSW && nxt < a.ntiles; cur ^= 1u;
            __syncthreads();
            continue;
        }
#endif
        if (!st.abn) for (uint32_t i = first_idx + rr_id; i < end_idx; i += 64 * RR) fast_group(st, tv, P, G, i);
        {
            const uint32_t nxt = next_of(t, cur);
            const bool draw = nxt < a.ntiles && nxt + gdim >= a.fast_dyn0;
            uint32_t tk = 0;
            if (draw && ticket_lane) tk = atomicAdd(a.fast_ticket, 1u);
            if (NSW && wave >= (uint32_t)(NWV - NSW) && nxt < a.ntiles)
                fast_scan<Cfg, (NSW ? NSW : 1)>(a, nxt, s_hit[cur ^ 1u], wave - (uint32_t)(NWV - NSW), lpt_a, own(wave - (uint32_t)(NWV - NSW), NSW, lpt_sw), tid & 63);
            if (draw && ticket_lane) s_next[cur ^ 1u] = a.fast_dyn0 + tk;
            scanned = NSW && nxt < a.ntiles; cur ^= 1u;
        }
        __syncthreads();
        STAMP(4);
        STOP_AFTER(4)
        STAMP(5);

        {
            auto& g = st.u.g;
            const uint32_t i = first_idx + tid;
            uint32_t cc = 0, cp = 0, cs = 0;
            uint32_t info = 0;
            if (i < NLe && !st.abn) {
                if (i < end_idx) {
                    info = g.g_info[i];
                    if (info & GI_START) cc += 1u;
                    if (info & GI_EMIT) cc += 1u << 10;
                    if ((info & GI_START) && (info & GI_COUNTER) == C_SELFCIRCLE) cc += 1u << 20;
                    cp = g.g_plen[i];
                }
                if (P.write_sam) cs = fast_line_sam(st, G, i);
            }
            uint32_t ec = cc, ep = cp, es = cs, tc, tp, ts;
            block_exscan3<NTW / 64>(ec, ep, es, tc, tp, ts, scan);
            if (tid == 0) {
                st.sums.groups = tc & 0x3FFu; st.sums.emitted = (tc >> 10) & 0x3FFu; st.sums.sc = (tc >> 20) & 0x3FFu;
                st.sums.pair_bytes = tp; st.sums.sam_bytes = ts;
                if (tp > 0xFFFFu) st.abn = AB_PAIR_BYTES;
                else if (!st.abn) {
                    const uint32_t e = claim_ranges(a, region, st.sums, st.base, st.region_pair0, st.region_sam0, s_out);
                    st.region_id = region;
                    if (e) lds_or(&st.abn, e << 8);
                    a.tile_groups[t] = (uint64_t)st.sums.groups | ((uint64_t)st.sums.emitted << 32);
                }
            }
            if (i < NLe && !(st.abn & 0xFFu)) {
                g.x_sam[i] = es;
                if (i < end_idx) {
                    g.x_grp[i] = (uint8_t)(ec & 0xFFu); g.x_sc[i] = (uint8_t)((ec >> 20) & 0xFFu); g.x_emit[i] = (uint8_t)((ec >> 10) & 0xFFu);
                    g.x_pair[i] = (uint16_t)(ep & 0xFFFFu);
                    if (info & GI_EMIT) g.em_idx[(ec >> 10) & 0xFFu] = (uint8_t)i;
                }
            }
        }
        __syncthreads();
        STAMP(6);
        STOP_AFTER(6)
        if (st.abn & 0xFFu) {
            if (tid == 0) {
                a.defer_list[atomicAdd(a.defer_count, 1u)] = t;
                const uint32_t why = st.abn & 0xFFu;
                if (why == AB_NO_PREV || why == AB_OPEN_GROUP) atomicAdd(a.defer_count + 1, 1u);
            }
#if defined(MKT_STAMPS)
            if (tid == 0 && a.stamps) { const uint32_t r = (st.abn & 0xFFu) - 1u; if (r < 12u) atomicAdd(&a.stamps[12 + r / 4u], 1ull << (16u * (r & 3u))); }
#endif
            __syncthreads();
            continue;
        }
        STAMP(7);
        STOP_AFTER(7)

        const uint32_t total = st.sums.pair_bytes;
        uint8_t* const dst = s_out.pairs + st.base.pair_bytes;
        for (uint32_t i = first_idx + ltid; i < end_idx; i += NTW) {
            fast_account(st, s_out, t, i);
            fast_last(st, G, &a.tile_last[t], i);
        }
        if (total && st.base.pair_bytes + total <= s_out.pairs_cap) {
            const auto& g = st.u.g;
            for (uint32_t e = (ltid + (uint32_t)(NTW / 2)) & (uint32_t)(NTW - 1); e < st.sums.emitted; e += NTW) {
                const uint32_t i = g.em_idx[e];
                fast_emit_line(st, g.g_slot[i], g.g_plen[i], dst + g.x_pair[i]);
            }
        }
        __syncthreads();
        STAMP(11);
        if (tid < (int)C_COUNT) wg_cnt[tid] += st.cnt[tid];
        if (tid == 0 && (st.abn >> 8)) atomicOr(&a.res->err, st.abn >> 8);
        const bool sam_copy = P.write_sam && st.sums.sam_bytes && st.base.sam_bytes + st.sums.sam_bytes <= s_out.sam_cap;
        uint32_t* eo = st.rc.f.pos;
        uint32_t* es = st.rc.f.rclip;
        uint32_t E = 0;
        if (sam_copy) {
            E = (uint32_t)(__popcll(st.m_emit[0]) + __popcll(st.m_emit[1]) + __popcll(st.m_emit[2]) + __popcll(st.m_emit[3]));
            for (uint32_t i = first_idx + (uint32_t)tid; i < NLe; i += NTW) {
                if (!mask_bit(st.m_emit, i)) continue;
                uint32_t k = (uint32_t)__popcll(st.m_emit[i >> 6] & ((1ull << (i & 63u)) - 1ull));
                for (uint32_t w = 0; w < (i >> 6); ++w) k += (uint32_t)__popcll(st.m_emit[w]);
                eo[k] = st.u.g.x_sam[i];
                es[k] = st.goff[i];
            }
            if (tid == 0) eo[E] = (uint32_t)st.sums.sam_bytes;
        }
        if (P.write_sam) __syncthreads();
        if (sam_copy && E) {
            const uint32_t total = (uint32_t)st.sums.sam_bytes;
            uint8_t* dbase = s_out.sam + st.base.sam_bytes;
            const uint8_t* tbase = a.text + G.w0;
            auto line_of = [&](uint32_t d) {
                uint32_t lo = 0, hi = E - 1u;
                while (lo < hi) { const uint32_t mid = (lo + hi + 1u) >> 1; if (eo[mid] <= d) lo = mid; else hi = mid - 1u; }
                return lo;
            };
            const uint32_t head0 = (uint32_t)((16u - ((uintptr_t)dbase & 15u)) & 15u);
            const uint32_t head = head0 < total ? head0 : total;
            const uint32_t nv = (total - head) >> 4, tail0 = head + (nv << 4);
            if ((uint32_t)tid < head) { const uint32_t k = line_of((uint32_t)tid); *MKT_GLOBAL(uint8_t, dbase + tid) = tbase[es[k] + (uint32_t)tid - eo[k]]; }
            if ((uint32_t)tid < total - tail0) { const uint32_t d = tail0 + (uint32_t)tid, k = line_of(d); *MKT_GLOBAL(uint8_t, dbase + d) = tbase[es[k] + d - eo[k]]; }
            for (uint32_t v = (uint32_t)tid; v < nv; v += NTW) {
                const uint32_t d = head + (v << 4);
                const uint32_t k = line_of(d);
                const uint32_t o = d - eo[k], left = eo[k + 1u] - d;
                const uint32_t so = es[k] + o;
                uint4 x;
                if (left >= 16u) __builtin_memcpy(&x, tbase + so, 16);
                else if (k + 2u <= E && eo[k + 2u] - eo[k + 1u] >= 16u - left && (uint64_t)G.w0 + so + 16u <= (uint64_t)n) {
                    uint4 xa, xb;
                    __builtin_memcpy(&xa, tbase + so, 16);
                    __builtin_memcpy(&xb, tbase + es[k + 1u] - left, 16);
                    const uint32_t* pa = reinterpret_cast<const uint32_t*>(&xa);
                    const uint32_t* pb = reinterpret_cast<const uint32_t*>(&xb);
                    uint32_t* px = reinterpret_cast<uint32_t*>(&x);
#pragma unroll
                    for (uint32_t q = 0; q < 4u; ++q) {
                        const uint32_t m = left >= 4u * q + 4u ? 0xFFFFFFFFu : (left <= 4u * q ? 0u : (1u << (8u * (left - 4u * q))) - 1u);
                        px[q] = (pa[q] & m) | (pb[q] & ~m);
                    }
                } else {
                    uint32_t q0 = 0, q1 = 0, q2 = 0, q3 = 0;
                    uint32_t kk = k, oo = so, lim = left;
#pragma unroll
                    for (uint32_t b2 = 0; b2 < 16u; ++b2) {
                        while (lim == 0u) { ++kk; oo = es[kk]; lim = eo[kk + 1u] - eo[kk]; }
                        const uint32_t by = (uint32_t)tbase[oo++] << (8u * (b2 & 3u));
                        if (b2 < 4u) q0 |= by; else if (b2 < 8u) q1 |= by; else if (b2 < 12u) q2 |= by; else q3 |= by;
                        --lim;
                    }
                    x = make_uint4(q0, q1, q2, q3);
                }
                *MKT_GLOBAL(uint4, dbase + d) = x;
            }
        }
        __syncthreads();
        STAMP(8);
    }
    if (tid0 < (int)C_COUNT && wg_cnt[tid0]) atomicAdd(&a.res->counters[tid0], wg_cnt[tid0]);
    STAMP_FLUSH(tid0);
    STAMP_SPAN(tid0);
}

constexpr int NTF = 1024;
__global__ __launch_bounds__(NTF) void k_finish_scan(KArgs a) {
    __shared__ uint64_t s_wave[NTF / 64];
    __shared__ uint64_t s_pre;
    __shared__ uint32_t s_chunk;
    const int tid = threadIdx.x, lane = tid & 63, wv = tid >> 6;
    if (tid == 0) s_chunk = atomicAdd(a.scan_ticket, 1u);
    __syncthreads();
    const uint32_t chunk = s_chunk;
    const uint32_t t = chunk * NTF + tid;
    const uint64_t x = t < a.ntiles ? a.tile_groups[t] : 0ull;
    if (t < a.ntiles && a.tile_last[t].valid) atomicMax(a.last_tile, (int)t + 1);
    uint64_t inc = x;
#pragma unroll
    for (int d = 1; d < 64; d <<= 1) { uint64_t y = shfl_up64(inc, d); if (lane >= d) inc += y; }
    if (lane == 63) s_wave[wv] = inc;
    __syncthreads();
    uint64_t pre = 0, tot = 0;
    for (int w = 0; w < NTF / 64; ++w) { if (w < wv) pre += s_wave[w]; tot += s_wave[w]; }
    if (wv == 0) {
        const uint64_t ex = lookback(a.scan_desc, chunk, ((tot & 0x7FFFFFFFull) << 31) | (tot >> 32), &a.res->err);
        if (lane == 0) s_pre = (ex >> 31) | ((ex & 0x7FFFFFFFull) << 32);
    }
    __syncthreads();
    if (t < a.ntiles) a.tile_groups[t] = s_pre + pre + inc - x;
    if (chunk == gridDim.x - 1 && tid == 0) a.res->groups = (s_pre + tot) & 0xFFFFFFFFull;
}

constexpr int kFinishGrid = 16;
__global__ __launch_bounds__(NTF) void k_finish(KArgs a) {
    const int tid = threadIdx.x;
    BlockResult* r = a.res;
    __shared__ uint64_t s_scpre[kMaxRegions + 1], s_ca[kMaxRegions], s_cb[kMaxRegions];
    __shared__ uint32_t s_err;
    if (tid < a.nregions) { s_ca[tid] = a.cur[tid].a; s_cb[tid] = a.cur[tid].b; }
    __syncthreads();
    if (tid == 0) {
        uint64_t pb = 0, em = 0, sb = 0, sc = 0;
        uint32_t err = 0;
        for (int q = 0; q < a.nregions; ++q) {
            const uint64_t ca = s_ca[q], cb = s_cb[q];
            const uint64_t p = ca & kCurLow, e = ca >> kCurShift, sm = cb & kCurLow, c = cb >> kCurShift;
            if (blockIdx.x == 0) { r->rpair[q] = p; r->rsam[q] = sm; }
            s_scpre[q] = sc;
            pb += p; em += e; sb += sm; sc += c;
            if (!a.ordered) {
                if (p > a.pairs_rcap) err |= E_PAIRS_CAP;
                if (sm > a.sam_rcap) err |= E_SAM_CAP;
                if (c > a.sc_rcap) err |= E_SC_CAP;
            }
        }
        s_scpre[a.nregions] = sc;
        if (a.ordered) { if (pb > a.out.pairs_cap) err |= E_PAIRS_CAP; if (sb > a.out.sam_cap) err |= E_SAM_CAP; if (sc > a.out.sc_cap) err |= E_SC_CAP; }
        if (a.run->sc + sc > a.sc_list_cap) err |= E_SC_CAP;
        if (a.keys_rcap && a.run->emitted + em > a.key_list_cap) err |= E_SC_CAP;
        s_err = err | r->err;
        if (blockIdx.x == 0) {
            r->pair_bytes = pb; r->emitted = em; r->sam_bytes = sb; r->sc = sc; r->nregions = (uint32_t)a.nregions;
            r->pad = a.defer_count ? *a.defer_count : 0u;
            r->pad2 = a.defer_count ? a.defer_count[1] : 0u;
            r->tiles = a.ntiles;
            const int last = *a.last_tile - 1;
            if (last >= 0) r->last = a.tile_last[last];
        }
    }
    __syncthreads();
    if (s_err == 0) {
        const uint64_t sc_base = a.run->sc, g_base = a.run->groups;
        const int nr = a.nregions;
        const int parts = (int)gridDim.x >= nr ? (int)gridDim.x / nr : 1;
        for (int q = (int)blockIdx.x % nr; q < nr; q += (int)gridDim.x) {
            const int part = (int)blockIdx.x / nr;
            if (part >= parts) break;
            const uint64_t cnt = s_scpre[q + 1] - s_scpre[q];
            const uint64_t* src = a.out.sc + (uint64_t)q * (a.ordered ? 0 : a.sc_rcap);
            for (uint64_t k = (uint64_t)part * NTF + tid; k < cnt; k += (uint64_t)parts * NTF) {
                const uint64_t e = src[k];
                a.sc_list[sc_base + s_scpre[q] + k] = g_base + (a.tile_groups[(uint32_t)(e >> 32)] & 0xFFFFFFFFull) + (uint32_t)(e & 0xFFFFFFFFu);
            }
        }
    }
    __syncthreads();
    if (blockIdx.x == 0 && tid == 0 && (s_err & ~r->err)) r->err |= s_err;
}

__global__ __launch_bounds__(256) void k_keys_place(KArgs a) {
    const BlockResult* r = a.res;
    if (r->err) return;
    __shared__ uint64_t pre[kMaxRegions + 1];
    if (threadIdx.x == 0) {
        uint64_t acc = 0;
        for (int q = 0; q < kMaxRegions; ++q) { pre[q] = acc; if (q < a.nregions) acc += a.cur[q].a >> kCurShift; }
        pre[kMaxRegions] = acc;
    }
    __syncthreads();
    const uint64_t base = a.run->emitted, total = pre[kMaxRegions];
    const uint64_t rstride = a.ordered ? 0 : a.keys_rcap;
    for (uint64_t x = (uint64_t)blockIdx.x * blockDim.x + threadIdx.x; x < total; x += (uint64_t)gridDim.x * blockDim.x) {
        uint32_t q = 0;
#pragma unroll
        for (uint32_t k = 1; k < (uint32_t)kMaxRegions; ++k) q += (x >= pre[k]) ? 1u : 0u;
        KeyRec rec = a.out.keys[(uint64_t)q * rstride + (x - pre[q])];
        const uint64_t ord = base + (a.tile_groups[(uint32_t)(rec.ord >> 16)] >> 32) + (rec.ord & 0xFFFFu);
        rec.ord = ord;
        a.key_list[ord] = rec;
    }
}
__global__ void k_run_advance(KArgs a) {
    BlockResult* r = a.res;
    if (threadIdx.x == 0 && r->err == 0) { a.run->groups += r->groups; a.run->sc += r->sc; a.run->emitted += r->emitted; }
}

struct GatherArgs {
    const BlockResult* res;
    const uint8_t* src; uint64_t rcap;
    uint8_t* dst; uint64_t dst_cap;
    int32_t which;
};
__global__ __launch_bounds__(256) void k_gather(GatherArgs g) {
    __shared__ uint64_t pre[kMaxRegions + 1];
    __shared__ uint64_t s_hole, s_tp;
    const BlockResult* r = g.res;
    if (r->err) return;
    if (threadIdx.x == 0) {
        const uint32_t nr = r->nregions ? r->nregions : 1u;
        uint64_t acc = 0;
        for (uint32_t q = 0; q < (uint32_t)kMaxRegions; ++q) { pre[q] = acc; if (q < nr) acc += g.which ? r->rsam[q] : r->rpair[q]; }
        pre[kMaxRegions] = acc;
        uint64_t tp = 0, hole = acc;
        if (r->last.valid) {
            tp = g.which ? r->last.sam_bytes : r->last.pair_bytes;
            const uint32_t lr = r->last.region < nr ? r->last.region : 0u;
            hole = pre[lr] + (g.which ? r->last.sam_off : r->last.pair_off);
        }
        s_hole = hole; s_tp = tp;
    }
    __syncthreads();
    const uint64_t total = pre[kMaxRegions], tp = s_tp, hole = s_hole, body = total - tp;
    if (total > g.dst_cap) return;
    auto src_of = [&](uint64_t x) -> const uint8_t* {
        const uint64_t y = x < body ? (x < hole ? x : x + tp) : hole + (x - body);
        uint32_t q = 0;
#pragma unroll
        for (uint32_t k = 1; k < (uint32_t)kMaxRegions; ++k) q += (y >= pre[k]) ? 1u : 0u;
        return g.src + (uint64_t)q * g.rcap + (y - pre[q]);
    };
    for (uint64_t x0 = ((uint64_t)blockIdx.x * blockDim.x + threadIdx.x) * 16u; x0 < total; x0 += (uint64_t)gridDim.x * blockDim.x * 16u) {
        const uint64_t x1 = x0 + 15u < total ? x0 + 15u : total - 1u;
        const uint8_t* a = src_of(x0);
        const uint8_t* b = src_of(x1);
        if (x1 - x0 == 15u && (uint64_t)(b - a) == 15u) {
            uint4 v;
            __builtin_memcpy(&v, a, 16);
            *reinterpret_cast<uint4*>(g.dst + x0) = v;
        } else {
            for (uint64_t x = x0; x <= x1; ++x) g.dst[x] = *src_of(x);
        }
    }
}
hipError_t launch_gather(const BlockResult* d_res, const uint8_t* src, uint64_t rcap, uint8_t* dst, uint64_t dst_cap, int which, uint64_t max_bytes, hipStream_t s) {
    GatherArgs g;
    g.res = d_res; g.src = src; g.rcap = rcap; g.dst = dst; g.dst_cap = dst_cap; g.which = which;
    uint64_t chunks = (max_bytes + 15) / 16;
    unsigned grid = (unsigned)((chunks + 255) / 256 < 2048 ? (chunks + 255) / 256 : 2048);
    if (grid == 0) grid = 1;
    hipLaunchKernelGGL(k_gather, dim3(grid), dim3(256), 0, s, g);
    return hipGetLastError();
}

__global__ void k_sc_logged(const uint64_t* list, uint64_t n, uint64_t drop_group, uint64_t group_offset, uint64_t K_total, uint32_t ref_threads,
                            unsigned long long* out) {
    unsigned long long mine = 0;
    for (uint64_t k = (uint64_t)blockIdx.x * blockDim.x + threadIdx.x; k < n; k += (uint64_t)gridDim.x * blockDim.x) {
        const uint64_t g = list[k];
        if (g == drop_group) continue;
        if (selfcircle_logged(group_offset + g, K_total, ref_threads)) ++mine;
    }
    for (int d = 32; d >= 1; d >>= 1) mine += shfl_xor64(mine, d);
    if ((threadIdx.x & 63) == 0 && mine) atomicAdd(out, mine);
}
hipError_t launch_sc_logged(const uint64_t* list, uint64_t n, uint64_t drop_group, uint64_t group_offset, uint64_t K_total, uint32_t ref_threads,
                            unsigned long long* out, hipStream_t s) {
    if (n == 0) return hipSuccess;
    const unsigned grid = (unsigned)((n + 255) / 256 < 1024 ? (n + 255) / 256 : 1024);
    hipLaunchKernelGGL(k_sc_logged, dim3(grid), dim3(256), 0, s, list, n, drop_group, group_offset, K_total, ref_threads, out);
    return hipGetLastError();
}

typedef FastCfg<kLeanTile, kLeanHB, kLeanHF, kLeanLCAP> CfgLean;
typedef TileCfg<kLeanTile, kLeanHB, kLeanHF, 512, 4> CfgFast;
typedef TileCfg<256, 64, 192, 512, 4> CfgSmall;

TileDims small_dims() { return cfg_dims<CfgSmall>(); }
TileDims max_dims() { return cfg_dims<CfgLean>(); }
static bool dims_ok(const TileDims& d, const TileDims& mx) {
    return d.tile >= 16u && !((d.tile | d.hb | d.hf) & 15u) && d.tile <= mx.tile && d.hb <= mx.hb && d.hf <= mx.hf;
}

uint32_t fast_max_workgroups(int) { return 256u * 4u; }

hipError_t launch_tiles(const KArgs& a, int cfg, int grid, hipStream_t s) {
    if (a.ntiles == 0) return hipSuccess;
    if (!dims_ok(a.dims, cfg == CFG_SMALL ? small_dims() : max_dims())) return hipErrorInvalidValue;
    if (cfg == CFG_SMALL) hipLaunchKernelGGL(k_tiles<CfgSmall>, dim3(grid), dim3(NT), 0, s, a);
    else hipLaunchKernelGGL(k_tiles<CfgFast>, dim3(grid), dim3(NT), 0, s, a);
    return hipGetLastError();
}
hipError_t launch_fast(const KArgs& a, int, int grid, hipStream_t s) {
    if (a.ntiles == 0) return hipSuccess;
    if (!dims_ok(a.dims, max_dims())) return hipErrorInvalidValue;
    hipLaunchKernelGGL((k_fast<CfgLean, NT, 2, 4>), dim3(grid), dim3(NT), 0, s, a);
    return hipGetLastError();
}
__global__ void k_count_nl(const uint8_t* text, size_t n, unsigned long long* out) {
    unsigned long long mine = 0;
    const size_t nv = n >> 4;
    for (size_t v = (size_t)blockIdx.x * blockDim.x + threadIdx.x; v < nv; v += (size_t)gridDim.x * blockDim.x) {
        const uint4 x = reinterpret_cast<const uint4*>(text)[v];
        mine += __popc(nl_flags(x.x)) + __popc(nl_flags(x.y)) + __popc(nl_flags(x.z)) + __popc(nl_flags(x.w));
    }
    if (blockIdx.x == 0 && threadIdx.x == 0) for (size_t b = nv << 4; b < n; ++b) mine += text[b] == '\n';
    for (int d = 32; d >= 1; d >>= 1) mine += shfl_xor64(mine, d);
    if ((threadIdx.x & 63) == 0 && mine) atomicAdd(out, mine);
}
hipError_t launch_count_newlines(const uint8_t* text, size_t n, unsigned long long* out, hipStream_t s) {
    if (n) hipLaunchKernelGGL(k_count_nl, dim3(64), dim3(256), 0, s, text, n, out);
    return hipGetLastError();
}
hipError_t launch_finish(const KArgs& a, hipStream_t s) {
    const unsigned chunks = (a.ntiles + NTF - 1) / NTF;
    if (chunks) hipLaunchKernelGGL(k_finish_scan, dim3(chunks), dim3(NTF), 0, s, a);
    hipLaunchKernelGGL(k_finish, dim3(kFinishGrid), dim3(NTF), 0, s, a);
    if (a.keys_rcap) hipLaunchKernelGGL(k_keys_place, dim3(2048), dim3(256), 0, s, a);
    hipLaunchKernelGGL(k_run_advance, dim3(1), dim3(64), 0, s, a);
    return hipGetLastError();
}
uint32_t finish_chunk_tiles() { return NTF; }

constexpr int DD_WG = 256;
constexpr int DS_WG = 512;
constexpr int DS_NW = DS_WG / 64;
constexpr int DS_T = 8192;
constexpr int DS_K = DS_T / DS_WG;
constexpr int DS_D = 7, DS_R = 1 << DS_D;
constexpr int DS_SCAN_WG = 1024, DS_SCAN_V = 8;
constexpr uint64_t kKeyMask1 = 0xFFFFFFFFC000FFFFull;
static_assert(DS_R == 2 * 64, "the scatter's prologue gives each lane of wave 0 two digits");

__device__ inline bool key_eq(const KeyRec& x, const KeyRec& y) { return x.k0 == y.k0 && (x.k1 & kKeyMask1) == (y.k1 & kKeyMask1); }

__global__ __launch_bounds__(DS_WG) void k_dd_prep(const KeyRec* keys, uint64_t n, int ib, uint64_t* rec, uint32_t* cnt, uint32_t G) {
    __shared__ uint32_t c[DS_R];
    if (threadIdx.x < DS_R) c[threadIdx.x] = 0;
    __syncthreads();
    const uint64_t b = (uint64_t)blockIdx.x * DS_T, e = b + DS_T < n ? b + DS_T : n, hi = ~((1ull << ib) - 1ull);
    for (uint64_t j = b + threadIdx.x; j < e; j += DS_WG) {
        const uint64_t r = (mix64(keys[j].k0 ^ mix64(keys[j].k1 & kKeyMask1)) & hi) | j;
        rec[j] = r;
        atomicAdd(&c[(r >> ib) & (DS_R - 1)], 1u);
    }
    __syncthreads();
    if (threadIdx.x < DS_R) cnt[threadIdx.x * G + blockIdx.x] = c[threadIdx.x];
}
__global__ __launch_bounds__(DS_WG) void k_dd_count(const uint64_t* rec, uint64_t n, int shift, uint32_t* cnt, uint32_t G) {
    __shared__ uint32_t c[DS_R];
    if (threadIdx.x < DS_R) c[threadIdx.x] = 0;
    __syncthreads();
    const uint64_t b = (uint64_t)blockIdx.x * DS_T, m = (b + DS_T < n ? b + DS_T : n) - b;
    const ulonglong2* v = reinterpret_cast<const ulonglong2*>(rec + b);
    for (uint64_t i = threadIdx.x; i < m / 2; i += DS_WG) {
        const ulonglong2 x = v[i];
        atomicAdd(&c[(x.x >> shift) & (DS_R - 1)], 1u);
        atomicAdd(&c[(x.y >> shift) & (DS_R - 1)], 1u);
    }
    if ((m & 1) && threadIdx.x == 0) atomicAdd(&c[(rec[b + m - 1] >> shift) & (DS_R - 1)], 1u);
    __syncthreads();
    if (threadIdx.x < DS_R) cnt[threadIdx.x * G + blockIdx.x] = c[threadIdx.x];
}
__global__ __launch_bounds__(DS_SCAN_WG) void k_dd_dscan(uint32_t* cnt, uint32_t G, uint32_t* tot) {
    __shared__ uint32_t wsum[DS_SCAN_WG / 64];
    const int lane = threadIdx.x & 63, wv = threadIdx.x >> 6;
    uint32_t* row = cnt + (uint64_t)blockIdx.x * G;
    uint32_t carry = 0;
    for (uint32_t base = 0; base < G; base += DS_SCAN_WG * DS_SCAN_V) {
        const uint32_t i0 = base + threadIdx.x * DS_SCAN_V;
        uint32_t v[DS_SCAN_V], s = 0;
#pragma unroll
        for (int k = 0; k < DS_SCAN_V; ++k) { v[k] = i0 + k < G ? row[i0 + k] : 0u; s += v[k]; }
        const uint32_t inc = wave_iscan32(s);
        if (lane == 63) wsum[wv] = inc;
        __syncthreads();
        uint32_t pre = carry, all = 0;
#pragma unroll
        for (int w = 0; w < DS_SCAN_WG / 64; ++w) { const uint32_t x = wsum[w]; if (w < wv) pre += x; all += x; }
        pre += inc - s;
#pragma unroll
        for (int k = 0; k < DS_SCAN_V; ++k) { if (i0 + k < G) row[i0 + k] = pre; pre += v[k]; }
        carry += all;
        __syncthreads();
    }
    if (threadIdx.x == 0) tot[blockIdx.x] = carry;
}
__global__ __launch_bounds__(DS_WG, 4) void k_dd_scatter(const uint64_t* rec, uint64_t n, int shift, const uint32_t* cnt, const uint32_t* tot, uint32_t G, uint64_t* rec2) {
    __shared__ uint64_t tile[DS_T];
    __shared__ uint32_t wrun[DS_NW][DS_R];
    __shared__ uint32_t gdelta[DS_R];
    const int tid = threadIdx.x, lane = tid & 63, wv = tid >> 6;
    const uint64_t b = (uint64_t)blockIdx.x * DS_T, m = (b + DS_T < n ? b + DS_T : n) - b;
    uint32_t gc0 = 0, gc1 = 0, t0 = 0, t1 = 0;
    if (wv == 0) {
        gc0 = cnt[(uint64_t)(2 * lane) * G + blockIdx.x]; gc1 = cnt[(uint64_t)(2 * lane + 1) * G + blockIdx.x];
        t0 = tot[2 * lane]; t1 = tot[2 * lane + 1];
    }
    for (int i = tid; i < DS_NW * DS_R; i += DS_WG) (&wrun[0][0])[i] = 0u;
    __syncthreads();
    uint64_t r[DS_K];
    uint32_t loc[DS_K / 2];
    const uint64_t lt = (1ull << lane) - 1ull;
#pragma unroll
    for (int k = 0; k < DS_K; ++k) {
        const uint64_t i = (uint64_t)wv * (DS_T / DS_NW) + k * 64 + lane;
        r[k] = i < m ? rec[b + i] : 0ull;
    }
#pragma unroll
    for (int k = 0; k < DS_K; ++k) {
        const uint64_t i = (uint64_t)wv * (DS_T / DS_NW) + k * 64 + lane;
        const bool live = i < m;
        const uint32_t d = (uint32_t)(r[k] >> shift) & (DS_R - 1);
        uint64_t peers = __ballot(live);
#pragma unroll
        for (int q = 0; q < DS_D; ++q) {
            const uint64_t s = __ballot((d >> q) & 1u);
            peers &= ((d >> q) & 1u) ? s : ~s;
        }
        const uint32_t before = wrun[wv][d];
        const uint32_t rk = before + (uint32_t)__popcll(peers & lt);
        loc[k / 2] = k & 1 ? loc[k / 2] | rk << 16 : rk;
        if (live && (peers & lt) == 0) wrun[wv][d] = before + (uint32_t)__popcll(peers);
    }
    __syncthreads();
    if (wv == 0) {
        uint32_t c0 = 0, c1 = 0;
        for (int w = 0; w < DS_NW; ++w) {
            const uint32_t x0 = wrun[w][2 * lane], x1 = wrun[w][2 * lane + 1];
            wrun[w][2 * lane] = c0; wrun[w][2 * lane + 1] = c1;
            c0 += x0; c1 += x1;
        }
        const uint32_t s = c0 + c1, ts = t0 + t1;
        const uint32_t e0 = wave_iscan32(s) - s, g0 = wave_iscan32(ts) - ts + gc0;
        const uint32_t e1 = e0 + c0, g1 = g0 + t0 - gc0 + gc1;
        for (int w = 0; w < DS_NW; ++w) { wrun[w][2 * lane] += e0; wrun[w][2 * lane + 1] += e1; }
        gdelta[2 * lane] = g0 - e0; gdelta[2 * lane + 1] = g1 - e1;
    }
    __syncthreads();
#pragma unroll
    for (int k = 0; k < DS_K; ++k) {
        const uint64_t i = (uint64_t)wv * (DS_T / DS_NW) + k * 64 + lane;
        if (i < m) tile[wrun[wv][(uint32_t)(r[k] >> shift) & (DS_R - 1)] + ((loc[k / 2] >> (16 * (k & 1))) & 0xFFFFu)] = r[k];
    }
    __syncthreads();
    for (uint32_t i = tid; i < m; i += DS_WG) {
        const uint64_t x = tile[i];
        rec2[gdelta[(uint32_t)(x >> shift) & (DS_R - 1)] + i] = x;
    }
}
__global__ __launch_bounds__(NT) void k_dd_scan(uint32_t* hist, uint32_t m) {
    __shared__ ScanScratch sc;
    __shared__ uint64_t carry;
    if (threadIdx.x == 0) carry = 0;
    __syncthreads();
    for (uint32_t base = 0; base < m; base += NT) {
        const uint32_t i = base + threadIdx.x;
        uint64_t x = i < m ? hist[i] : 0, d = 0, tx, td, e = x;
        block_exscan2(e, d, tx, td, sc);
        if (i < m) hist[i] = (uint32_t)(carry + e);
        __syncthreads();
        if (threadIdx.x == 0) carry += tx;
        __syncthreads();
    }
}
__global__ __launch_bounds__(256) void k_dd_mark(const KeyRec* keys, const uint64_t* rec, uint64_t n, int ib, uint64_t run_mask, uint8_t* flags, DedupResult* res) {
    const uint64_t imask = (1ull << ib) - 1ull, j = (uint64_t)blockIdx.x * blockDim.x + threadIdx.x;
    bool dup = false;
    if (j < n) {
        const uint64_t r = rec[j];
        uint64_t o = j ? rec[j - 1] : ~r;
        bool have = false;
        KeyRec me;
        for (uint64_t b = j - 1; !((o ^ r) & run_mask);) {
            if (!((o ^ r) >> ib)) {
                if (!have) { me = keys[r & imask]; have = true; }
                if (key_eq(keys[o & imask], me)) { dup = true; break; }
            }
            if (b-- == 0) break;
            o = rec[b];
        }
        if (dup) flags[r & imask] = 1;
    }
    const uint64_t m = __ballot(dup);
    if ((threadIdx.x & 63) == 0 && m) atomicAdd((unsigned long long*)&res->dups, (unsigned long long)__popcll(m));
    if (blockIdx.x == 0 && threadIdx.x == 0) res->total = n;
}
size_t dedup_work_bytes(uint64_t n) {
    const uint64_t G = (n + DS_T - 1) / DS_T;
    return (size_t)(n * (8 + 8) + DS_R * (G + 1) * 4 + 4096);
}
hipError_t launch_dedup(const KeyRec* keys, uint64_t n, uint8_t* flags, void* work, size_t work_bytes, DedupResult* d_res, hipStream_t s) {
    hipError_t e = hipMemsetAsync(d_res, 0, sizeof(DedupResult), s);
    if (e != hipSuccess || n == 0) return e;
    if (work_bytes < dedup_work_bytes(n) || n >= (1ull << 32)) return hipErrorInvalidValue;
    const uint32_t G = (uint32_t)((n + DS_T - 1) / DS_T);
    uint8_t* w = (uint8_t*)(((uintptr_t)work + 255) & ~(uintptr_t)255);
    uint64_t* rA = (uint64_t*)w; w += ((n * 8 + 255) & ~255ull);
    uint64_t* rB = (uint64_t*)w; w += ((n * 8 + 255) & ~255ull);
    uint32_t* cnt = (uint32_t*)w;
    uint32_t* tot = cnt + (uint64_t)DS_R * G;
    int ib = 1;
    while ((1ull << ib) < n) ++ib;
    int bits = 2;
    while (bits < 34 && (1ull << (bits - 2)) < n) ++bits;
    bits = bits < 12 ? 12 : (bits > 32 ? 32 : bits);
    const int passes = (bits + DS_D - 1) / DS_D;
    const int sorted = passes * DS_D < 64 - ib ? passes * DS_D : 64 - ib;
    hipLaunchKernelGGL(k_dd_prep, dim3(G), dim3(DS_WG), 0, s, keys, n, ib, rA, cnt, G);
    for (int p = 0; p < passes; ++p) {
        if (p) hipLaunchKernelGGL(k_dd_count, dim3(G), dim3(DS_WG), 0, s, (const uint64_t*)rA, n, ib + DS_D * p, cnt, G);
        hipLaunchKernelGGL(k_dd_dscan, dim3(DS_R), dim3(DS_SCAN_WG), 0, s, cnt, G, tot);
        hipLaunchKernelGGL(k_dd_scatter, dim3(G), dim3(DS_WG), 0, s, (const uint64_t*)rA, n, ib + DS_D * p, (const uint32_t*)cnt, (const uint32_t*)tot, G, rB);
        uint64_t* t = rA; rA = rB; rB = t;
    }
    const uint64_t run_mask = ((1ull << sorted) - 1ull) << ib;
    e = hipMemsetAsync(flags, 0, n, s);
    if (e != hipSuccess) return e;
    hipLaunchKernelGGL(k_dd_mark, dim3((unsigned)((n + 255) / 256)), dim3(256), 0, s, keys, (const uint64_t*)rA, n, ib, run_mask, flags, d_res);
    return hipGetLastError();
}
size_t radix64_count_bytes(uint64_t n) { return (size_t)(DS_R * ((n + DS_T - 1) / DS_T + 1) * 4 + 4096); }
hipError_t launch_radix64(uint64_t*& rA, uint64_t*& rB, uint64_t n, int lo_bit, int nbits, uint32_t* cnt, hipStream_t s) {
    if (n == 0 || nbits <= 0) return hipSuccess;
    if (n >= (1ull << 32) || lo_bit < 0 || lo_bit + nbits > 64) return hipErrorInvalidValue;
    const uint32_t G = (uint32_t)((n + DS_T - 1) / DS_T);
    uint32_t* tot = cnt + (uint64_t)DS_R * G;
    for (int sh = lo_bit; sh < lo_bit + nbits; sh += DS_D) {
        hipLaunchKernelGGL(k_dd_count, dim3(G), dim3(DS_WG), 0, s, (const uint64_t*)rA, n, sh, cnt, G);
        hipLaunchKernelGGL(k_dd_dscan, dim3(DS_R), dim3(DS_SCAN_WG), 0, s, cnt, G, tot);
        hipLaunchKernelGGL(k_dd_scatter, dim3(G), dim3(DS_WG), 0, s, (const uint64_t*)rA, n, sh, (const uint32_t*)cnt, (const uint32_t*)tot, G, rB);
        uint64_t* t = rA; rA = rB; rB = t;
    }
    return hipGetLastError();
}

constexpr uint32_t kMaxWorld = 16;
__device__ inline KeyRec part_remap(KeyRec r, const uint16_t* lut) {
    if (lut) {
        const uint64_t a = lut[(r.k0 >> 45) & (kChrSlots - 1u)], b = lut[(r.k0 >> 32) & (kChrSlots - 1u)];
        r.k0 = (a << 45) | (b << 32) | (r.k0 & 0xFFFFFFFFull);
    }
    return r;
}
__device__ inline uint32_t part_dest(const KeyRec& r, uint32_t world) { return (uint32_t)(mix64(r.k0 ^ mix64(r.k1 & kKeyMask1)) % world); }
__global__ __launch_bounds__(DD_WG) void k_part_hist(const KeyRec* keys, uint64_t n, uint64_t per, const uint16_t* lut, uint32_t world, uint32_t* hist, uint32_t G) {
    __shared__ uint32_t cnt[kMaxWorld];
    if (threadIdx.x < kMaxWorld) cnt[threadIdx.x] = 0;
    __syncthreads();
    const uint64_t b = (uint64_t)blockIdx.x * per, e = b + per < n ? b + per : n;
    for (uint64_t j = b + threadIdx.x; j < e; j += DD_WG) atomicAdd(&cnt[part_dest(part_remap(keys[j], lut), world)], 1u);
    __syncthreads();
    if (threadIdx.x < kMaxWorld) hist[threadIdx.x * G + blockIdx.x] = cnt[threadIdx.x];
}
__global__ __launch_bounds__(DD_WG) void k_part_scatter(const KeyRec* keys, uint64_t n, uint64_t per, const uint16_t* lut, uint32_t world, const uint32_t* hist,
                                                       uint32_t G, KeyRec* send, uint32_t* perm) {
    __shared__ uint32_t base[kMaxWorld];
    __shared__ uint32_t wcnt[DD_WG / 64][kMaxWorld];
    const int tid = threadIdx.x, lane = tid & 63, wv = tid >> 6;
    if (tid < (int)kMaxWorld) base[tid] = hist[tid * G + blockIdx.x];
    __syncthreads();
    const uint64_t b = (uint64_t)blockIdx.x * per, e = b + per < n ? b + per : n;
    for (uint64_t j0 = b; j0 < e; j0 += DD_WG) {
        const uint64_t j = j0 + tid;
        const bool live = j < e;
        KeyRec r;
        r.k0 = r.k1 = r.ord = 0;
        if (live) r = part_remap(keys[j], lut);
        const uint32_t d = live ? part_dest(r, world) : kMaxWorld;
        uint32_t rank = 0;
        for (uint32_t dd = 0; dd < world; ++dd) {
            const uint64_t m = __ballot(d == dd);
            if (d == dd) rank = __popcll(m & ((1ull << lane) - 1ull));
            if (lane == 0) wcnt[wv][dd] = __popcll(m);
        }
        __syncthreads();
        if (live) {
            uint32_t o = base[d] + rank;
            for (int w = 0; w < wv; ++w) o += wcnt[w][d];
            send[o] = r;
            perm[j] = o;
        }
        __syncthreads();
        if (tid < (int)world) { uint32_t s2 = 0; for (int w = 0; w < DD_WG / 64; ++w) s2 += wcnt[w][tid]; base[tid] += s2; }
        __syncthreads();
    }
}
__global__ void k_unpermute_flags(const uint8_t* in, const uint32_t* perm, uint64_t n, uint8_t* out, unsigned long long* dups) {
    uint32_t mine = 0;
    for (uint64_t j = (uint64_t)blockIdx.x * blockDim.x + threadIdx.x; j < n; j += (uint64_t)gridDim.x * blockDim.x) {
        const uint8_t f = in[perm[j]];
        out[j] = f;
        mine += f ? 1u : 0u;
    }
    if (mine) atomicAdd(dups, (unsigned long long)mine);
}
size_t partition_work_bytes() { return (size_t)(kMaxWorld * 1024 + 64) * 4; }
hipError_t launch_partition(const KeyRec* keys, uint64_t n, const uint16_t* d_lut, uint32_t world, uint32_t* hist, KeyRec* send, uint32_t* perm, uint32_t* G_out, hipStream_t s) {
    if (world == 0 || world > kMaxWorld || n >= (1ull << 32)) return hipErrorInvalidValue;
    uint32_t G = (uint32_t)((n + 8191) / 8192);
    if (G > 1024) G = 1024;
    if (G == 0) G = 1;
    *G_out = G;
    const uint64_t per = (n + G - 1) / G;
    hipError_t e = hipMemsetAsync(hist, 0, (size_t)kMaxWorld * G * 4, s);
    if (e != hipSuccess || n == 0) return e;
    hipLaunchKernelGGL(k_part_hist, dim3(G), dim3(DD_WG), 0, s, keys, n, per, d_lut, world, hist, G);
    hipLaunchKernelGGL(k_dd_scan, dim3(1), dim3(NT), 0, s, hist, kMaxWorld * G);
    hipLaunchKernelGGL(k_part_scatter, dim3(G), dim3(DD_WG), 0, s, keys, n, per, d_lut, world, (const uint32_t*)hist, G, send, perm);
    return hipGetLastError();
}
hipError_t launch_unpermute(const uint8_t* in, const uint32_t* perm, uint64_t n, uint8_t* out, unsigned long long* dups, hipStream_t s) {
    hipError_t e = hipMemsetAsync(dups, 0, sizeof(unsigned long long), s);
    if (e != hipSuccess || n == 0) return e;
    hipLaunchKernelGGL(k_unpermute_flags, dim3(1024), dim3(256), 0, s, in, perm, n, out, dups);
    return hipGetLastError();
}

__global__ __launch_bounds__(256) void k_chrstat(const KeyRec* keys, uint64_t n, const uint16_t* dense_of_slot, uint32_t ndense, unsigned long long* counts) {
    __shared__ uint32_t loc[32 * 32];
    for (int k = threadIdx.x; k < 1024; k += 256) loc[k] = 0;
    __syncthreads();
    for (uint64_t j = (uint64_t)blockIdx.x * blockDim.x + threadIdx.x; j < n; j += (uint64_t)gridDim.x * blockDim.x) {
        const uint64_t k0 = keys[j].k0;
        const uint32_t a = dense_of_slot[(k0 >> 45) & (kChrSlots - 1u)], b = dense_of_slot[(k0 >> 32) & (kChrSlots - 1u)];
        if (a < 32u && b < 32u) atomicAdd(&loc[a * 32u + b], 1u);
        else atomicAdd(&counts[(uint64_t)a * ndense + b], 1ull);
    }
    __syncthreads();
    for (int k = threadIdx.x; k < 1024; k += 256) {
        const uint32_t a = k >> 5, b = k & 31;
        if (loc[k] && a < ndense && b < ndense) atomicAdd(&counts[(uint64_t)a * ndense + b], (unsigned long long)loc[k]);
    }
}
hipError_t launch_chrstat(const KeyRec* keys, uint64_t n, const uint16_t* dense_of_slot, uint32_t ndense, unsigned long long* counts, hipStream_t s) {
    if (n) hipLaunchKernelGGL(k_chrstat, dim3(512), dim3(256), 0, s, keys, n, dense_of_slot, ndense, counts);
    return hipGetLastError();
}

__global__ void k_synth_sizes(SynParams p, uint64_t first, uint64_t n, uint64_t* sizes) {
    uint64_t i = (uint64_t)blockIdx.x * blockDim.x + threadIdx.x;
    if (i >= n) return;
    SynCountSink c;
    synth_group(c, p, first + i);
    sizes[i] = c.n;
}
__global__ void k_synth_write(SynParams p, uint64_t first, uint64_t n, const uint64_t* offs, char* out) {
    uint64_t i = (uint64_t)blockIdx.x * blockDim.x + threadIdx.x;
    if (i >= n) return;
    SynMemSink m{out + offs[i]};
    synth_group(m, p, first + i);
}
__global__ void k_exscan_u64(uint64_t* v, uint64_t n, uint64_t* total) {
    __shared__ ScanScratch sc;
    __shared__ uint64_t carry;
    if (threadIdx.x == 0) carry = 0;
    __syncthreads();
    for (uint64_t base = 0; base < n; base += NT) {
        uint64_t i = base + threadIdx.x;
        uint64_t x = i < n ? v[i] : 0, d = 0, tx, td;
        uint64_t e = x;
        block_exscan2(e, d, tx, td, sc);
        if (i < n) v[i] = carry + e;
        __syncthreads();
        if (threadIdx.x == 0) carry += tx;
        __syncthreads();
    }
    if (threadIdx.x == 0) *total = carry;
}
__global__ void k_synth_tail(SynParams p, char* out) {
    if (threadIdx.x == 0 && blockIdx.x == 0) { SynMemSink m{out}; synth_tail_group(m, p); }
}

hipError_t launch_synth_sizes(const SynParams& p, uint64_t first, uint64_t n, uint64_t* sizes, hipStream_t s) {
    if (n) hipLaunchKernelGGL(k_synth_sizes, dim3((unsigned)((n + 255) / 256)), dim3(256), 0, s, p, first, n, sizes);
    return hipGetLastError();
}
constexpr uint32_t XS_PER = 16 * NT;
__global__ __launch_bounds__(NT) void k_xs_sums(const uint64_t* v, uint64_t n, uint64_t* part) {
    __shared__ uint64_t sh[NT / 64];
    const uint64_t b = (uint64_t)blockIdx.x * XS_PER;
    uint64_t x = 0;
    for (uint32_t k = 0; k < XS_PER / NT; ++k) { const uint64_t i = b + k * NT + threadIdx.x; if (i < n) x += v[i]; }
#pragma unroll
    for (int d = 32; d >= 1; d >>= 1) x += shfl_xor64(x, d);
    if ((threadIdx.x & 63) == 0) sh[threadIdx.x >> 6] = x;
    __syncthreads();
    if (threadIdx.x == 0) { uint64_t t = 0; for (int w = 0; w < NT / 64; ++w) t += sh[w]; part[blockIdx.x] = t; }
}
__global__ __launch_bounds__(NT) void k_xs_apply(uint64_t* v, uint64_t n, const uint64_t* part) {
    __shared__ ScanScratch sc;
    __shared__ uint64_t carry;
    if (threadIdx.x == 0) carry = part[blockIdx.x];
    __syncthreads();
    const uint64_t b = (uint64_t)blockIdx.x * XS_PER;
    for (uint32_t k = 0; k < XS_PER / NT; ++k) {
        const uint64_t i = b + k * NT + threadIdx.x;
        uint64_t e = i < n ? v[i] : 0, d = 0, tx, td;
        block_exscan2(e, d, tx, td, sc);
        if (i < n) v[i] = carry + e;
        __syncthreads();
        if (threadIdx.x == 0) carry += tx;
        __syncthreads();
    }
}
hipError_t launch_exscan(uint64_t* v, uint64_t n, uint64_t* total, hipStream_t s) {
    if (n <= 4 * XS_PER) {
        hipLaunchKernelGGL(k_exscan_u64, dim3(1), dim3(NT), 0, s, v, n, total);
        return hipGetLastError();
    }
    const uint64_t nb = (n + XS_PER - 1) / XS_PER;
    uint64_t* part = nullptr;
    hipError_t e = hipMallocAsync((void**)&part, (nb + 1) * sizeof(uint64_t), s);
    if (e != hipSuccess) return e;
    hipLaunchKernelGGL(k_xs_sums, dim3((unsigned)nb), dim3(NT), 0, s, (const uint64_t*)v, n, part);
    hipLaunchKernelGGL(k_exscan_u64, dim3(1), dim3(NT), 0, s, part, nb, total);
    hipLaunchKernelGGL(k_xs_apply, dim3((unsigned)nb), dim3(NT), 0, s, v, n, (const uint64_t*)part);
    e = hipGetLastError();
    const hipError_t e2 = hipFreeAsync(part, s);
    return e != hipSuccess ? e : e2;
}
hipError_t launch_synth_write(const SynParams& p, uint64_t first, uint64_t n, const uint64_t* offs, char* out, hipStream_t s) {
    if (n) hipLaunchKernelGGL(k_synth_write, dim3((unsigned)((n + 255) / 256)), dim3(256), 0, s, p, first, n, offs, out);
    return hipGetLastError();
}
hipError_t launch_synth_tail(const SynParams& p, char* out, hipStream_t s) {
    hipLaunchKernelGGL(k_synth_tail, dim3(1), dim3(64), 0, s, p, out);
    return hipGetLastError();
}
size_t synth_tail_bytes(const SynParams& p) {
    SynCountSink c;
    synth_tail_group(c, p);
    return c.n;
}

}
```

### microcket_amd/csrc/mkt_launch.h

```cpp
#pragma once
#include <hip/hip_runtime.h>
#include "mkt_host.h"
#include "mkt_fast.h"
#include "mkt_synth.h"

namespace mkt {

enum { CFG_FAST = 0, CFG_SMALL = 1 };

struct DevRun { uint64_t groups, sc, emitted; };

struct alignas(128) RegionCur { unsigned long long a, b; unsigned long long pad[14]; };
constexpr int kMaxRegions = 16;
constexpr int kCurShift = 36;
constexpr unsigned long long kCurLow = (1ull << kCurShift) - 1ull;

constexpr uint32_t kFastAllStatic = 0xFFFFFFFFu;
struct KArgs {
    const uint8_t* text;
    uint32_t n;
    uint32_t ntiles;
    TileDims dims;
    uint32_t fast_dyn0;
    Params P;
    uint64_t* descA;
    uint64_t* descB;
    uint64_t* descC;
    uint32_t* ticket;
    uint32_t* fast_ticket;
    uint64_t* tile_groups;
    int32_t ordered;
    TileLast* tile_last;
    uint32_t* defer_list;
    uint32_t* defer_count;
    int* last_tile;
    uint64_t* scan_desc;
    uint32_t* scan_ticket;
    int32_t use_list;
    BlockResult* res;
    DevRun* run;
    RegionCur* cur;
    int32_t nregions;
    uint64_t pairs_rcap, sam_rcap, sc_rcap;
    uint64_t* sc_list;
    uint64_t sc_list_cap;
    uint64_t keys_rcap;
    KeyRec* key_list;
    uint64_t key_list_cap;
    OutPtrs out;
    unsigned long long* stamps;
    int32_t debug_stop;
};

struct BlockWs {
    uint8_t* base;
    uint32_t ntiles;
    static constexpr size_t kScanWords = 1024;
    size_t tiles_bytes() const { return ((size_t)ntiles * (3 * sizeof(uint64_t) + sizeof(TileLast) + sizeof(uint64_t) + sizeof(uint32_t)) + 127) & ~(size_t)127; }
    size_t bytes() const { return tiles_bytes() + kMaxRegions * sizeof(RegionCur) + 256 + kScanWords * sizeof(uint64_t) + sizeof(BlockResult); }
    uint64_t* descA() const { return (uint64_t*)base; }
    uint64_t* descB() const { return descA() + ntiles; }
    uint64_t* descC() const { return descB() + ntiles; }
    TileLast* tile_last() const { return (TileLast*)(descC() + ntiles); }
    uint64_t* tile_groups() const { return (uint64_t*)(tile_last() + ntiles); }
    uint32_t* defer_list() const { return (uint32_t*)(tile_groups() + ntiles); }
    RegionCur* cur() const { return (RegionCur*)(base + tiles_bytes()); }
    uint8_t* counters() const { return (uint8_t*)(cur() + kMaxRegions); }
    uint32_t* ticket() const { return (uint32_t*)counters(); }
    uint32_t* defer_count() const { return (uint32_t*)(counters() + 64); }
    uint32_t* defer_ticket() const { return (uint32_t*)(counters() + 128); }
    uint32_t* fast_ticket() const { return (uint32_t*)(counters() + 160); }
    int* last_tile() const { return (int*)(counters() + 192); }
    uint32_t* scan_ticket() const { return (uint32_t*)(counters() + 224); }
    uint64_t* scan_desc() const { return (uint64_t*)(counters() + 256); }
    BlockResult* res() const { return (BlockResult*)(scan_desc() + kScanWords); }
};

TileDims small_dims();
TileDims max_dims();
uint32_t fast_max_workgroups(int cfg);
hipError_t launch_count_newlines(const uint8_t* text, size_t n, unsigned long long* out, hipStream_t s);
hipError_t launch_tiles(const KArgs& a, int cfg, int grid, hipStream_t s);
hipError_t launch_fast(const KArgs& a, int cfg, int grid, hipStream_t s);
uint32_t finish_chunk_tiles();
hipError_t launch_finish(const KArgs& a, hipStream_t s);
hipError_t launch_gather(const BlockResult* d_res, const uint8_t* src, uint64_t rcap, uint8_t* dst, uint64_t dst_cap, int which, uint64_t max_bytes, hipStream_t s);
hipError_t launch_sc_logged(const uint64_t* list, uint64_t n, uint64_t drop_group, uint64_t group_offset, uint64_t K_total, uint32_t ref_threads,
                            unsigned long long* out, hipStream_t s);

struct DedupResult { uint64_t total, dups; };
hipError_t launch_dedup(const KeyRec* keys, uint64_t n, uint8_t* flags, void* work, size_t work_bytes, DedupResult* d_res, hipStream_t s);
size_t dedup_work_bytes(uint64_t n);
size_t radix64_count_bytes(uint64_t n);
hipError_t launch_radix64(uint64_t*& rA, uint64_t*& rB, uint64_t n, int lo_bit, int nbits, uint32_t* cnt, hipStream_t s);
size_t partition_work_bytes();
hipError_t launch_partition(const KeyRec* keys, uint64_t n, const uint16_t* d_lut, uint32_t world, uint32_t* hist, KeyRec* send, uint32_t* perm, uint32_t* G_out, hipStream_t s);
hipError_t launch_unpermute(const uint8_t* in, const uint32_t* perm, uint64_t n, uint8_t* out, unsigned long long* dups, hipStream_t s);
hipError_t launch_chrstat(const KeyRec* keys, uint64_t n, const uint16_t* dense_of_slot, uint32_t ndense, unsigned long long* counts, hipStream_t s);

hipError_t launch_synth_sizes(const SynParams& p, uint64_t first, uint64_t n, uint64_t* sizes, hipStream_t s);
hipError_t launch_exscan(uint64_t* v, uint64_t n, uint64_t* total, hipStream_t s);
hipError_t launch_synth_write(const SynParams& p, uint64_t first, uint64_t n, const uint64_t* offs, char* out, hipStream_t s);
hipError_t launch_synth_tail(const SynParams& p, char* out, hipStream_t s);
size_t synth_tail_bytes(const SynParams& p);

}
```

Baseline: 2.250 billion read-pairs/s.

## Batch per-block epilogue kernels across up to eight blocks per launch

Blocks in the lean path now run their fast kernel immediately but defer the deferred-tile, finish-scan, finish, key-placement and run-advance epilogue. Up to eight blocks are then processed together by batched kernels indexed by blockIdx.y, each block using its own workspace bank and output buffers. Running-total offsets are rebuilt on the device from the earlier blocks in the batch. The goal is to cut per-block launch count, small kernels and result copies, at the cost of extra device memory for the banks, flushes at every sync point, and more complex error and replay handling.

```diff
diff --git a/microcket_amd/csrc/mkt_capi.cpp b/microcket_amd/csrc/mkt_capi.cpp
--- a/microcket_amd/csrc/mkt_capi.cpp
+++ b/microcket_amd/csrc/mkt_capi.cpp
@@ -1,4 +1,22 @@
 #include "mkt_ctx.h"
+
+int flush_batch(mkt_ctx* c) {
+    const uint32_t nb = c->pend_n;
+    if (!nb) return MKT_OK;
+    c->pend_n = 0;
+    if (nb == 1) {
+        const KArgs& b = c->pend.a[0];
+        HIPCHK(c, launch_tiles(b, CFG_FAST, b.ntiles < 96u ? (int)b.ntiles : 96, c->stream));
+        HIPCHK(c, launch_finish(b, c->stream));
+        HIPCHK(c, hipMemcpyAsync(&c->h_res[c->pend_slot0], b.res, sizeof(BlockResult), hipMemcpyDeviceToHost, c->stream));
+        return MKT_OK;
+    }
+    c->pend.nb = nb;
+    c->pend.res_out = (BlockResult*)(c->d_ws + (size_t)c->batch_g * c->ws_stride);
+    HIPCHK(c, launch_epilogue_batch(c->pend, c->stream));
+    HIPCHK(c, hipMemcpyAsync(&c->h_res[c->pend_slot0], c->pend.res_out, nb * sizeof(BlockResult), hipMemcpyDeviceToHost, c->stream));
+    return MKT_OK;
+}
 
 extern "C" {
 
@@ -58,6 +76,12 @@
         else if (e[0] && end && !*end && v < 0xFFFFFFFFul) c->fast_rounds = (uint32_t)v;
         else { mkt_destroy(c); return fail(nullptr, MKT_E_ARG, "MKT_FAST_ROUNDS must be a number of rounds or \"all\""); }
     }
+    if (const char* e = getenv("MKT_EPILOGUE_BATCH")) {
+        char* end = nullptr;
+        const unsigned long v = strtoul(e, &end, 10);
+        if (e[0] && end && !*end && v >= 1 && v <= (unsigned long)kMaxBatch) c->batch_g = (uint32_t)v;
+        else { mkt_destroy(c); return fail(nullptr, MKT_E_ARG, "MKT_EPILOGUE_BATCH must be a number of blocks from 1 to %d", kMaxBatch); }
+    }
     size_t bc = p->block_bytes ? (size_t)p->block_bytes : ((size_t)64 << 20);
     if (bc < 4096) bc = 4096;
     if (bc >= kMaxBlock) bc = kMaxBlock - 4096;
@@ -82,6 +106,7 @@
         c->cv.notify_all();
         c->worker.join();
     }
+    (void)flush_batch(c);
     (void)sync_all(c);
     delete c;
 }
@@ -143,14 +168,46 @@
     if (((uintptr_t)d_text & 15u) != 0) return fail(c, MKT_E_ARG, "block text must be 16-byte aligned");
     if (n >= kMaxBlock) return fail(c, MKT_E_ARG, "block of %zu bytes: must be < 2 GiB - 64 KiB", n);
     const uint32_t ntiles = num_tiles((uint32_t)n, dims.tile);
+    if ((ntiles + finish_chunk_tiles() - 1) / finish_chunk_tiles() > BlockWs::kScanWords) return fail(c, MKT_E_ARG, "block has too many tiles for the finish scan");
     BlockWs ws{nullptr, ntiles};
     const size_t ws_bytes = ws.bytes();
-    int rc = ensure(c, c->d_ws, ws_bytes, ws_bytes + ws_bytes / 4, true);
-    if (rc) return rc;
-    ws.base = c->d_ws;
-    if ((ntiles + finish_chunk_tiles() - 1) / finish_chunk_tiles() > BlockWs::kScanWords) return fail(c, MKT_E_ARG, "block has too many tiles for the finish scan");
-    if ((rc = ensure_dev(c, c->d_pairs, n / 3 + 65536))) return rc;
-    if (c->P.write_sam && (rc = ensure_dev(c, c->d_sam, n + n / 4 + 65536))) return rc;
+    int rc;
+    if (c->p.extensions & MKT_EXT_KEYS) {
+        const double per_byte = c->key_density > 0 ? (c->key_density * 2 < 1.0 / 64 ? c->key_density * 2 : 1.0 / 64) : 1.0 / 64;
+        const size_t want = (size_t)c->acc.emitted + (size_t)((double)(c->bytes_unsynced + n) * per_byte) + 65536;
+        if (!c->d_key_list.fits(want)) {
+            size_t ncap = c->d_key_list.cap() ? c->d_key_list.cap() * 2 : ((size_t)1 << 22);
+            while (ncap < want) ncap *= 2;
+            if ((rc = flush_batch(c))) return rc;
+            HIPCHK(c, hipStreamSynchronize(c->stream));
+            HIPCHK(c, c->d_key_list.regrow_keep(ncap, c->d_key_list.cap()));
+        }
+    }
+    const bool lean = !c->p.ordered && cfg != CFG_SMALL && !c->no_lean;
+    const bool batched = !so && lean && c->batch_g > 1;
+    uint32_t bank = 0;
+    if (!batched) {
+        if ((rc = flush_batch(c))) return rc;
+        if ((rc = ensure(c, c->d_ws, ws_bytes, ws_bytes + ws_bytes / 4, true))) return rc;
+        ws.base = c->d_ws;
+    } else {
+        if (c->pend_n && (ws_bytes > c->ws_stride || slot != c->pend_slot0 + c->pend_n) && (rc = flush_batch(c))) return rc;
+        bank = c->pend_n;
+        if (bank == 0) {
+            if (ws_bytes > c->ws_stride) c->ws_stride = (ws_bytes + ws_bytes / 4 + 255) & ~(size_t)255;
+            c->pend_limit = c->probing && slot == 0 ? 1u : c->batch_g;
+            c->pend_slot0 = slot;
+            const size_t all = (size_t)c->batch_g * c->ws_stride + kMaxBatch * sizeof(BlockResult);
+            if ((rc = ensure(c, c->d_ws, all, all, true))) return rc;
+        }
+        ws.base = c->d_ws + (size_t)bank * c->ws_stride;
+    }
+    GrowBuf<uint8_t>& d_pairs = bank ? c->banks[bank - 1].d_pairs : c->d_pairs;
+    GrowBuf<uint8_t>& d_sam = bank ? c->banks[bank - 1].d_sam : c->d_sam;
+    GrowBuf<uint64_t>& d_sc_tmp = bank ? c->banks[bank - 1].d_sc_tmp : c->d_sc_tmp;
+    GrowBuf<KeyRec>& d_keys_raw = bank ? c->banks[bank - 1].d_keys_raw : c->d_keys_raw;
+    if ((rc = ensure_dev(c, d_pairs, n / 3 + 65536))) return rc;
+    if (c->P.write_sam && (rc = ensure_dev(c, d_sam, n + n / 4 + 65536))) return rc;
     if (!c->d_sc && (rc = ensure_sc_list(c, 1))) return rc;
     KArgs a;
     memset(&a, 0, sizeof a);
@@ -165,28 +222,20 @@
     a.run = c->d_run;
     a.nregions = c->p.ordered ? 1 : kMaxRegions;
     const size_t sc_need = (size_t)a.nregions * ((n / 256 / (size_t)a.nregions) * 2 + 1024);
-    if ((rc = ensure(c, c->d_sc_tmp, sc_need, sc_need, true))) return rc;
-    a.pairs_rcap = (c->d_pairs.cap() / a.nregions) & ~(uint64_t)15;
-    a.sam_rcap = c->P.write_sam ? ((c->d_sam.cap() / a.nregions) & ~(uint64_t)15) : 0;
-    a.sc_rcap = c->d_sc_tmp.cap() / a.nregions;
-    a.out.pairs = c->d_pairs; a.out.pairs_cap = c->d_pairs.cap();
-    a.out.sam = c->d_sam; a.out.sam_cap = c->P.write_sam ? c->d_sam.cap() : 0;
-    a.out.sc = c->d_sc_tmp; a.out.sc_cap = c->d_sc_tmp.cap();
+    if ((rc = ensure(c, d_sc_tmp, sc_need, sc_need, true))) return rc;
+    a.pairs_rcap = (d_pairs.cap() / a.nregions) & ~(uint64_t)15;
+    a.sam_rcap = c->P.write_sam ? ((d_sam.cap() / a.nregions) & ~(uint64_t)15) : 0;
+    a.sc_rcap = d_sc_tmp.cap() / a.nregions;
+    a.out.pairs = d_pairs; a.out.pairs_cap = d_pairs.cap();
+    a.out.sam = d_sam; a.out.sam_cap = c->P.write_sam ? d_sam.cap() : 0;
+    a.out.sc = d_sc_tmp; a.out.sc_cap = d_sc_tmp.cap();
     a.sc_list = c->d_sc; a.sc_list_cap = c->d_sc.cap();
     if (c->p.extensions & MKT_EXT_KEYS) {
         if (!c->d_chr) { HIPCHK(c, c->d_chr.alloc(1)); HIPCHK(c, hipMemsetAsync(c->d_chr, 0, sizeof(ChrTab), c->stream)); }
         const size_t per = (n / 64 / (size_t)a.nregions) * 2 + 4096, need = per * a.nregions;
-        if ((rc = ensure(c, c->d_keys_raw, need, need, true))) return rc;
-        const double per_byte = c->key_density > 0 ? (c->key_density * 2 < 1.0 / 64 ? c->key_density * 2 : 1.0 / 64) : 1.0 / 64;
-        const size_t want = (size_t)c->acc.emitted + (size_t)((double)(c->bytes_unsynced + n) * per_byte) + 65536;
-        if (!c->d_key_list.fits(want)) {
-            size_t ncap = c->d_key_list.cap() ? c->d_key_list.cap() * 2 : ((size_t)1 << 22);
-            while (ncap < want) ncap *= 2;
-            HIPCHK(c, hipStreamSynchronize(c->stream));
-            HIPCHK(c, c->d_key_list.regrow_keep(ncap, c->d_key_list.cap()));
-        }
-        a.keys_rcap = c->d_keys_raw.cap() / a.nregions;
-        a.out.keys = c->d_keys_raw; a.out.keys_cap = c->d_keys_raw.cap(); a.out.chr = c->d_chr;
+        if ((rc = ensure(c, d_keys_raw, need, need, true))) return rc;
+        a.keys_rcap = d_keys_raw.cap() / a.nregions;
+        a.out.keys = d_keys_raw; a.out.keys_cap = d_keys_raw.cap(); a.out.chr = c->d_chr;
         a.out.key_lanes = (c->p.extensions & MKT_EXT_LANES) ? 1u : 0u;
         a.key_list = c->d_key_list; a.key_list_cap = c->d_key_list.cap();
     }
@@ -195,7 +244,8 @@
     a.stamps = getenv("MKT_NO_STAMPS") ? nullptr : c->d_stamps;
     { const char* e = getenv("MKT_DEBUG_STOP"); a.debug_stop = e ? atoi(e) : 0; }
 #endif
-    HIPCHK(c, hipMemsetAsync(c->d_ws, 0, ws_bytes, c->stream));
+    if (!batched) HIPCHK(c, hipMemsetAsync(c->d_ws, 0, ws_bytes, c->stream));
+    else if (bank == 0) HIPCHK(c, hipMemsetAsync(c->d_ws, 0, (size_t)c->pend_limit * c->ws_stride, c->stream));
     hipEvent_t e0, e1;
     if (so) { e0 = so->k0; e1 = so->k1; }
     else {
@@ -214,13 +264,18 @@
 #if defined(MKT_STAMPS)
     if (a.debug_stop) a.fast_dyn0 = kFastAllStatic;
 #endif
-    const bool lean = !c->p.ordered && cfg != CFG_SMALL && !c->no_lean;
+    c->last_bank = bank; c->last_ws_off = (size_t)(ws.base - c->d_ws.get());
     HIPCHK(c, hipEventRecord(e0, c->stream));
     if (lean) {
         HIPCHK(c, launch_fast(a, cfg, grid, c->stream));
         HIPCHK(c, hipEventRecord(e1, c->stream));
         KArgs b = a;
         b.use_list = 1; b.ticket = ws.defer_ticket();
+        if (batched) {
+            c->pend.a[bank] = b;
+            ++c->pend_n;
+            return c->pend_n >= c->pend_limit ? flush_batch(c) : MKT_OK;
+        }
         HIPCHK(c, launch_tiles(b, cfg, ntiles < 96u ? (int)ntiles : 96, c->stream));
     } else {
         HIPCHK(c, launch_tiles(a, cfg, grid, c->stream));
@@ -689,11 +744,12 @@
     const bool dbg = getenv("MKT_DEBUG_SYNC") != nullptr;
     auto now = [] { return std::chrono::duration<double, std::milli>(std::chrono::steady_clock::now().time_since_epoch()).count(); };
     const double t0 = dbg ? now() : 0;
+    int rc = flush_batch(c);
+    if (rc) return rc;
     HIPCHK(c, hipStreamSynchronize(c->stream));
     const double t1 = dbg ? now() : 0;
     fold_timing(c);
     const double t2 = dbg ? now() : 0;
-    int rc = MKT_OK;
     bool changed = false;
     int replays = 0;
     for (size_t k = c->res_folded; k < c->res_used; ++k) {
@@ -707,6 +763,7 @@
                 changed = true;
                 if ((rc = rewind_run(c))) return rc;
                 for (size_t j = k; j < c->res_used; ++j) if ((rc = enqueue_block(c, c->res_text[j], c->res_n[j], c->cfg, c->dims, j))) return rc;
+                if ((rc = flush_batch(c))) return rc;
                 HIPCHK(c, hipStreamSynchronize(c->stream));
                 fold_timing(c);
                 --k;
@@ -731,23 +788,26 @@
 int mkt_fetch_last_block(mkt_ctx* c, char* pairs, size_t pairs_cap, size_t* pairs_len, char* sam, size_t sam_cap, size_t* sam_len) {
     if (!c) return MKT_E_ARG;
     HIPCHK(c, hipSetDevice(c->p.device));
+    { const int rc = flush_batch(c); if (rc) return rc; }
     HIPCHK(c, hipStreamSynchronize(c->stream));
     BlockResult r;
     const uint32_t ntiles = num_tiles((uint32_t)c->last_n, c->last_dims.tile ? c->last_dims.tile : c->dims.tile);
-    HIPCHK(c, hipMemcpy(&r, BlockWs{c->d_ws, ntiles}.res(), sizeof r, hipMemcpyDeviceToHost));
+    HIPCHK(c, hipMemcpy(&r, BlockWs{c->d_ws + c->last_ws_off, ntiles}.res(), sizeof r, hipMemcpyDeviceToHost));
+    const GrowBuf<uint8_t>& d_pairs = c->last_bank ? c->banks[c->last_bank - 1].d_pairs : c->d_pairs;
+    const GrowBuf<uint8_t>& d_sam = c->last_bank ? c->banks[c->last_bank - 1].d_sam : c->d_sam;
     if (pairs_len) *pairs_len = (size_t)r.pair_bytes;
     if (sam_len) *sam_len = c->P.write_sam ? (size_t)r.sam_bytes : 0;
     const uint32_t nreg = r.nregions ? r.nregions : 1;
-    const size_t prc = (c->d_pairs.cap() / nreg) & ~(size_t)15, src_ = c->P.write_sam ? ((c->d_sam.cap() / nreg) & ~(size_t)15) : 0;
+    const size_t prc = (d_pairs.cap() / nreg) & ~(size_t)15, src_ = c->P.write_sam ? ((d_sam.cap() / nreg) & ~(size_t)15) : 0;
     if (pairs && r.pair_bytes) {
         if (pairs_cap < r.pair_bytes) return fail(c, MKT_E_ARG, "pairs buffer too small (%llu needed)", (unsigned long long)r.pair_bytes);
         size_t acc = 0;
-        for (uint32_t q = 0; q < nreg; ++q) { if (r.rpair[q]) HIPCHK(c, hipMemcpy(pairs + acc, c->d_pairs + (size_t)q * prc, (size_t)r.rpair[q], hipMemcpyDeviceToHost)); acc += (size_t)r.rpair[q]; }
+        for (uint32_t q = 0; q < nreg; ++q) { if (r.rpair[q]) HIPCHK(c, hipMemcpy(pairs + acc, d_pairs + (size_t)q * prc, (size_t)r.rpair[q], hipMemcpyDeviceToHost)); acc += (size_t)r.rpair[q]; }
     }
     if (sam && c->P.write_sam && r.sam_bytes) {
         if (sam_cap < r.sam_bytes) return fail(c, MKT_E_ARG, "sam buffer too small (%llu needed)", (unsigned long long)r.sam_bytes);
         size_t acc = 0;
-        for (uint32_t q = 0; q < nreg; ++q) { if (r.rsam[q]) HIPCHK(c, hipMemcpy(sam + acc, c->d_sam + (size_t)q * src_, (size_t)r.rsam[q], hipMemcpyDeviceToHost)); acc += (size_t)r.rsam[q]; }
+        for (uint32_t q = 0; q < nreg; ++q) { if (r.rsam[q]) HIPCHK(c, hipMemcpy(sam + acc, d_sam + (size_t)q * src_, (size_t)r.rsam[q], hipMemcpyDeviceToHost)); acc += (size_t)r.rsam[q]; }
     }
     return MKT_OK;
 }
@@ -802,6 +862,7 @@
         for (int i = 0; i < mkt_ctx::kOut; ++i) { c->outs[i].dev_busy = false; c->outs[i].host_busy = false; }
         c->async_rc = MKT_OK; c->cur = 0; c->seq = 0; c->consumer_async = false;
     }
+    (void)flush_batch(c);
     HIPCHK(c, hipStreamSynchronize(c->stream));
     fold_timing(c);
     HIPCHK(c, hipMemsetAsync(c->d_run, 0, sizeof(DevRun), c->stream));
diff --git a/microcket_amd/csrc/mkt_capi_util.cpp b/microcket_amd/csrc/mkt_capi_util.cpp
--- a/microcket_amd/csrc/mkt_capi_util.cpp
+++ b/microcket_amd/csrc/mkt_capi_util.cpp
@@ -141,6 +141,7 @@
 int mkt_copy_to_host(mkt_ctx* c, const void* d_src, void* dst, size_t n) {
     if (!c || !d_src || !dst) return MKT_E_ARG;
     HIPCHK(c, hipSetDevice(c->p.device));
+    { const int rc = flush_batch(c); if (rc) return rc; }
     HIPCHK(c, hipMemcpy(dst, d_src, n, hipMemcpyDeviceToHost));
     return MKT_OK;
 }
diff --git a/microcket_amd/csrc/mkt_ctx.h b/microcket_amd/csrc/mkt_ctx.h
--- a/microcket_amd/csrc/mkt_ctx.h
+++ b/microcket_amd/csrc/mkt_ctx.h
@@ -22,6 +22,7 @@
 
 static const size_t kMaxBlock = ((size_t)1 << 31) - 65536;
 static const uint32_t kFastRoundsDefault = 8;
+static const uint32_t kEpilogueBatchDefault = 8;
 static const size_t kStampWords = 20;
 
 inline thread_local std::string g_create_error;
@@ -52,6 +53,14 @@
     GrowBuf<KeyRec> d_key_list;
     DevBuf<ChrTab> d_chr;
     GrowBuf<uint8_t> d_ws;
+    struct Bank { GrowBuf<uint8_t> d_pairs, d_sam; GrowBuf<uint64_t> d_sc_tmp; GrowBuf<KeyRec> d_keys_raw; };
+    Bank banks[kMaxBatch - 1];
+    uint32_t batch_g = kEpilogueBatchDefault;
+    KBatch pend;
+    uint32_t pend_n = 0, pend_limit = 1;
+    size_t pend_slot0 = 0;
+    size_t ws_stride = 0;
+    uint32_t last_bank = 0; size_t last_ws_off = 0;
     DevBuf<DevRun> d_run;
     size_t h_len = 0;
     PinBuf<BlockResult> h_res; size_t res_slots = 0, res_used = 0, res_folded = 0;
@@ -129,6 +138,7 @@
     HIPCHK(c, buf.regrow(new_cap));
     return MKT_OK;
 }
+int flush_batch(mkt_ctx* c);
 inline uint64_t ext_key_count(mkt_ctx* c, int drop_last) {
     uint64_t n = c->acc.emitted;
     if (drop_last && c->acc.pending.valid && c->acc.pending.pair_bytes && n) --n;
diff --git a/microcket_amd/csrc/mkt_kernels.hip b/microcket_amd/csrc/mkt_kernels.hip
--- a/microcket_amd/csrc/mkt_kernels.hip
+++ b/microcket_amd/csrc/mkt_kernels.hip
@@ -201,7 +201,7 @@
 }
 
 template <class Cfg>
-__global__ __launch_bounds__(NT) void k_tiles(KArgs a) {
+__device__ __forceinline__ void tiles_body(const KArgs& a) {
     __shared__ TileState<Cfg> st;
     __shared__ ScanScratch scan;
     __shared__ uint32_t s_tile;
@@ -405,6 +405,14 @@
         __syncthreads();
     }
     STAMP_FLUSH(tid);
+}
+template <class Cfg>
+__global__ __launch_bounds__(NT) void k_tiles(KArgs a) { tiles_body<Cfg>(a); }
+template <class Cfg>
+__global__ __launch_bounds__(NT) void k_tiles_batch(KBatch b) {
+    const KArgs a = b.a[blockIdx.y];
+    if (blockIdx.x >= *a.defer_count) return;
+    tiles_body<Cfg>(a);
 }
 
 constexpr int kLoadBatch = 14;
@@ -826,7 +834,7 @@
 }
 
 constexpr int NTF = 1024;
-__global__ __launch_bounds__(NTF) void k_finish_scan(KArgs a) {
+__device__ __forceinline__ void finish_scan_body(const KArgs& a, uint32_t nchunks) {
     __shared__ uint64_t s_wave[NTF / 64];
     __shared__ uint64_t s_pre;
     __shared__ uint32_t s_chunk;
@@ -850,11 +858,18 @@
     }
     __syncthreads();
     if (t < a.ntiles) a.tile_groups[t] = s_pre + pre + inc - x;
-    if (chunk == gridDim.x - 1 && tid == 0) a.res->groups = (s_pre + tot) & 0xFFFFFFFFull;
+    if (chunk == nchunks - 1 && tid == 0) a.res->groups = (s_pre + tot) & 0xFFFFFFFFull;
+}
+__global__ __launch_bounds__(NTF) void k_finish_scan(KArgs a) { finish_scan_body(a, gridDim.x); }
+__global__ __launch_bounds__(NTF) void k_finish_scan_batch(KBatch b) {
+    const KArgs a = b.a[blockIdx.y];
+    const uint32_t nchunks = (a.ntiles + NTF - 1) / NTF;
+    if (blockIdx.x >= nchunks) return;
+    finish_scan_body(a, nchunks);
 }
 
 constexpr int kFinishGrid = 16;
-__global__ __launch_bounds__(NTF) void k_finish(KArgs a) {
+__device__ __forceinline__ void finish_body(const KArgs& a, const DevRun& run) {
     const int tid = threadIdx.x;
     BlockResult* r = a.res;
     __shared__ uint64_t s_scpre[kMaxRegions + 1], s_ca[kMaxRegions], s_cb[kMaxRegions];
@@ -878,8 +893,8 @@
         }
         s_scpre[a.nregions] = sc;
         if (a.ordered) { if (pb > a.out.pairs_cap) err |= E_PAIRS_CAP; if (sb > a.out.sam_cap) err |= E_SAM_CAP; if (sc > a.out.sc_cap) err |= E_SC_CAP; }
-        if (a.run->sc + sc > a.sc_list_cap) err |= E_SC_CAP;
-        if (a.keys_rcap && a.run->emitted + em > a.key_list_cap) err |= E_SC_CAP;
+        if (run.sc + sc > a.sc_list_cap) err |= E_SC_CAP;
+        if (a.keys_rcap && run.emitted + em > a.key_list_cap) err |= E_SC_CAP;
         s_err = err | r->err;
         if (blockIdx.x == 0) {
             r->pair_bytes = pb; r->emitted = em; r->sam_bytes = sb; r->sc = sc; r->nregions = (uint32_t)a.nregions;
@@ -892,7 +907,7 @@
     }
     __syncthreads();
     if (s_err == 0) {
-        const uint64_t sc_base = a.run->sc, g_base = a.run->groups;
+        const uint64_t sc_base = run.sc, g_base = run.groups;
         const int nr = a.nregions;
         const int parts = (int)gridDim.x >= nr ? (int)gridDim.x / nr : 1;
         for (int q = (int)blockIdx.x % nr; q < nr; q += (int)gridDim.x) {
@@ -909,6 +924,28 @@
     __syncthreads();
     if (blockIdx.x == 0 && tid == 0 && (s_err & ~r->err)) r->err |= s_err;
 }
+__global__ __launch_bounds__(NTF) void k_finish(KArgs a) { finish_body(a, *a.run); }
+__global__ __launch_bounds__(NTF) void k_finish_batch(KBatch b) {
+    __shared__ unsigned long long s_pre[3];
+    const int tid = threadIdx.x;
+    const uint32_t j = blockIdx.y;
+    if (tid < 3) s_pre[tid] = 0;
+    __syncthreads();
+    if ((uint32_t)tid < j * (uint32_t)kMaxRegions) {
+        const KArgs& e = b.a[tid / kMaxRegions];
+        const int q = tid % kMaxRegions;
+        if (q < e.nregions) {
+            atomicAdd(&s_pre[1], e.cur[q].b >> kCurShift);
+            atomicAdd(&s_pre[2], e.cur[q].a >> kCurShift);
+        }
+        if (q == 0) atomicAdd(&s_pre[0], (unsigned long long)e.res->groups);
+    }
+    __syncthreads();
+    const KArgs a = b.a[j];
+    DevRun run = *a.run;
+    run.groups += s_pre[0]; run.sc += s_pre[1]; run.emitted += s_pre[2];
+    finish_body(a, run);
+}
 
 __global__ __launch_bounds__(256) void k_keys_place(KArgs a) {
     const BlockResult* r = a.res;
@@ -935,6 +972,59 @@
 __global__ void k_run_advance(KArgs a) {
     BlockResult* r = a.res;
     if (threadIdx.x == 0 && r->err == 0) { a.run->groups += r->groups; a.run->sc += r->sc; a.run->emitted += r->emitted; }
+}
+
+constexpr int kKeysPlaceWG = NT;
+__global__ __launch_bounds__(kKeysPlaceWG) void k_keys_place_batch(KBatch b) {
+    __shared__ uint64_t pre[kMaxBatch * kMaxRegions + 1];
+    __shared__ ScanScratch scan;
+    __shared__ const KeyRec* s_keys[kMaxBatch];
+    __shared__ const uint64_t* s_tg[kMaxBatch];
+    __shared__ uint64_t s_rstride[kMaxBatch];
+    __shared__ uint32_t s_skip[kMaxBatch];
+    const uint32_t tid = threadIdx.x, nb = b.nb;
+    static_assert(kMaxBatch * kMaxRegions < kKeysPlaceWG, "one lane per block and region, and one behind them for the total");
+    uint64_t cnt = 0, dummy = 0, total, td;
+    if (tid < nb * (uint32_t)kMaxRegions) {
+        const KArgs& e = b.a[tid / kMaxRegions];
+        const int q = (int)(tid % kMaxRegions);
+        if (q < e.nregions) cnt = e.cur[q].a >> kCurShift;
+        if (q == 0) {
+            s_keys[tid / kMaxRegions] = e.out.keys; s_tg[tid / kMaxRegions] = e.tile_groups;
+            s_rstride[tid / kMaxRegions] = e.ordered ? 0 : e.keys_rcap; s_skip[tid / kMaxRegions] = e.res->err;
+        }
+    }
+    block_exscan2(cnt, dummy, total, td, scan);
+    if (tid <= nb * (uint32_t)kMaxRegions) pre[tid] = cnt;
+    __syncthreads();
+    const uint64_t base = b.a[0].run->emitted;
+    for (uint64_t x = (uint64_t)blockIdx.x * blockDim.x + tid; x < total; x += (uint64_t)gridDim.x * blockDim.x) {
+        uint32_t j = 0, q = 0;
+#pragma unroll
+        for (uint32_t k = 1; k < (uint32_t)kMaxBatch; ++k) j += (k < nb && x >= pre[k * kMaxRegions]) ? 1u : 0u;
+        if (s_skip[j]) continue;
+        const uint64_t* pj = pre + j * kMaxRegions;
+#pragma unroll
+        for (uint32_t k = 1; k < (uint32_t)kMaxRegions; ++k) q += (x >= pj[k]) ? 1u : 0u;
+        KeyRec rec = s_keys[j][(uint64_t)q * s_rstride[j] + (x - pj[q])];
+        const uint64_t ord = base + pj[0] + (s_tg[j][(uint32_t)(rec.ord >> 16)] >> 32) + (rec.ord & 0xFFFFu);
+        rec.ord = ord;
+        b.a[0].key_list[ord] = rec;
+    }
+}
+__global__ __launch_bounds__(64 * kMaxBatch) void k_run_advance_batch(KBatch b) {
+    constexpr uint32_t W = sizeof(BlockResult) / sizeof(uint64_t);
+    static_assert(sizeof(BlockResult) % sizeof(uint64_t) == 0 && W <= 64, "a result is copied by one wave, a word per lane");
+    const uint32_t j = threadIdx.x >> 6, w = threadIdx.x & 63;
+    if (j < b.nb && w < W) reinterpret_cast<uint64_t*>(b.res_out + j)[w] = reinterpret_cast<const uint64_t*>(b.a[j].res)[w];
+    if (threadIdx.x == 0) {
+        DevRun* run = b.a[0].run;
+        for (uint32_t k = 0; k < b.nb; ++k) {
+            const BlockResult* r = b.a[k].res;
+            if (r->err) break;
+            run->groups += r->groups; run->sc += r->sc; run->emitted += r->emitted;
+        }
+    }
 }
 
 struct GatherArgs {
@@ -1062,6 +1152,24 @@
     return hipGetLastError();
 }
 uint32_t finish_chunk_tiles() { return NTF; }
+hipError_t launch_epilogue_batch(const KBatch& b, hipStream_t s) {
+    if (b.nb == 0 || b.nb > (uint32_t)kMaxBatch) return hipErrorInvalidValue;
+    uint32_t max_tiles = 0;
+    for (uint32_t j = 0; j < b.nb; ++j) {
+        const KArgs& a = b.a[j];
+        if (a.ntiles && !dims_ok(a.dims, max_dims())) return hipErrorInvalidValue;
+        if (a.run != b.a[0].run || a.key_list != b.a[0].key_list || !a.keys_rcap != !b.a[0].keys_rcap) return hipErrorInvalidValue;
+        if (a.ntiles > max_tiles) max_tiles = a.ntiles;
+    }
+    const unsigned chunks = (max_tiles + NTF - 1) / NTF;
+    const unsigned per = (96u + b.nb - 1) / b.nb;
+    if (max_tiles) hipLaunchKernelGGL(k_tiles_batch<CfgFast>, dim3(max_tiles < per ? max_tiles : per, b.nb), dim3(NT), 0, s, b);
+    if (chunks) hipLaunchKernelGGL(k_finish_scan_batch, dim3(chunks, b.nb), dim3(NTF), 0, s, b);
+    hipLaunchKernelGGL(k_finish_batch, dim3(kFinishGrid, b.nb), dim3(NTF), 0, s, b);
+    if (b.a[0].keys_rcap) hipLaunchKernelGGL(k_keys_place_batch, dim3(2048), dim3(kKeysPlaceWG), 0, s, b);
+    hipLaunchKernelGGL(k_run_advance_batch, dim3(1), dim3(64 * kMaxBatch), 0, s, b);
+    return hipGetLastError();
+}
 
 constexpr int DD_WG = 256;
 constexpr int DS_WG = 512;
diff --git a/microcket_amd/csrc/mkt_launch.h b/microcket_amd/csrc/mkt_launch.h
--- a/microcket_amd/csrc/mkt_launch.h
+++ b/microcket_amd/csrc/mkt_launch.h
@@ -76,6 +76,13 @@
     BlockResult* res() const { return (BlockResult*)(scan_desc() + kScanWords); }
 };
 
+constexpr int kMaxBatch = 8;
+struct KBatch {
+    KArgs a[kMaxBatch];
+    BlockResult* res_out;
+    uint32_t nb;
+};
+
 TileDims small_dims();
 TileDims max_dims();
 uint32_t fast_max_workgroups(int cfg);
@@ -83,6 +90,7 @@
 hipError_t launch_tiles(const KArgs& a, int cfg, int grid, hipStream_t s);
 hipError_t launch_fast(const KArgs& a, int cfg, int grid, hipStream_t s);
 uint32_t finish_chunk_tiles();
+hipError_t launch_epilogue_batch(const KBatch& b, hipStream_t s);
 hipError_t launch_finish(const KArgs& a, hipStream_t s);
 hipError_t launch_gather(const BlockResult* d_res, const uint8_t* src, uint64_t rcap, uint8_t* dst, uint64_t dst_cap, int which, uint64_t max_bytes, hipStream_t s);
 hipError_t launch_sc_logged(const uint64_t* list, uint64_t n, uint64_t drop_group, uint64_t group_offset, uint64_t K_total, uint32_t ref_threads,
```

After: 2.333 billion read-pairs/s (median of 6 runs). 3.7% higher.
